# avik-pal/RegNeuralDE.jl

Hardware: AMD Instinct MI355X
Metric: training-step samples/sec + mean NFE, MNIST Neural ODE bs=512 (higher is better)
Workload: dtype f32; 1 GPU; MNIST NODE regularized (error_est), Tsit5 reltol=abstol=1.4e-8, batch 512 per GPU, 1xMI355X per rank; step = loss fwd + reverse pass through the solver + InvDecay/Momentum update; the weights train during the timed steps (mean_nfe drifts with --steps: value_fixed_weights of --full is the stationary companion); global_batch=512, parallelism=single

## Files before the change

### include/rnde.h

```cpp
#ifndef RNDE_H
#define RNDE_H
#include <stddef.h>
#include <stdint.h>

#ifdef __cplusplus
extern "C" {
#endif

#define RNDE_MAX_LAYERS 8

typedef enum {
    RNDE_OK = 0,
    RNDE_ERR_BAD_ARG = 1,
    RNDE_ERR_MAX_ATTEMPTS = 2,
    RNDE_ERR_DT_UNDERFLOW = 3,
    RNDE_ERR_NONFINITE = 4,
    RNDE_ERR_HIP = 5,
    RNDE_ERR_NO_TAPE = 6,
    RNDE_ERR_NO_DEVICE = 7
} rnde_status;

typedef enum { RNDE_ACT_IDENTITY = 0, RNDE_ACT_TANH = 1, RNDE_ACT_RELU = 2, RNDE_ACT_SIGMOID = 3, RNDE_ACT_SOFTPLUS = 4, RNDE_ACT_ELU = 5 } rnde_act;
typedef enum { RNDE_PRE_NONE = 0, RNDE_PRE_TANH = 1, RNDE_PRE_CUBE = 2 } rnde_pre_act;
typedef enum { RNDE_SOLVER_TSIT5 = 0, RNDE_SOLVER_DP5 = 1, RNDE_SOLVER_DOP853 = 2 } rnde_solver;
// ... 21 lines not shown
    int32_t wgrad_side_pct;
    int32_t stage_generic;
} rnde_node_config;

typedef struct rnde_node rnde_node;
typedef struct rnde_comm rnde_comm;

const char* rnde_version(void);
int64_t     rnde_debug_poison_allocs(void);
int64_t     rnde_debug_poison_bytes(void);
int64_t     rnde_debug_live_allocs(void);
int64_t     rnde_debug_live_bytes(void);
const char* rnde_last_error(const rnde_node* h);
int32_t     rnde_param_count(const rnde_node_config* cfg);

rnde_status rnde_node_create(const rnde_node_config* cfg, rnde_node** out);
void        rnde_node_destroy(rnde_node* h);

rnde_status rnde_node_create_tiled(const rnde_node_config* cfg, rnde_node** out);
int64_t     rnde_node_tiled_lds_bytes(const rnde_node_config* cfg);

rnde_status rnde_node_set_tracking(rnde_node* h, int32_t track_ctrl, int32_t track_initdt);
rnde_status rnde_node_tracking(const rnde_node* h, int32_t* ctrl_out, int32_t* initdt_out);

rnde_status rnde_node_tiled_reserve_saveat(rnde_node* h, int32_t max_saveat);
int32_t     rnde_node_tiled_saveat_capacity(const rnde_node* h);

rnde_status rnde_node_forward(rnde_node* h, const float* x_dev, const float* p_dev, int32_t B,
                              float t0, float t1, float* u_out_dev, int64_t* nfe_out,
                              float* saveval_host, int32_t* n_saveval_out, int32_t keep_tape,
                              void* stream);

rnde_status rnde_node_forward_saveat(rnde_node* h, const float* x_dev, const float* p_dev, int32_t B,
                                     float t0, float t1, const float* saveat_host, int32_t n_saveat,
                                     float* u_saved_dev, int64_t* nfe_out, float* saveval_host,
                                     int32_t* n_saveval_out, int32_t keep_tape, void* stream);

rnde_status rnde_node_forward_everystep(rnde_node* h, const float* x_dev, const float* p_dev, int32_t B, float t0, float t1,
                                        int32_t save_start, float* sol_out_dev, int32_t capacity, float* t_host_out, int32_t* n_out,
                                        int64_t* nfe_out, float* saveval_host, int32_t* n_saveval_out, int32_t keep_tape, void* stream);

rnde_status rnde_node_forward_replay(rnde_node* h, const float* x_dev, const float* p_dev, int32_t B,
                                     float t0, float t1, const float* steps_host, int32_t n_steps,
                                     float* u_out_dev, int64_t* nfe_out, float* saveval_host,
                                     int32_t* n_saveval_out, int32_t keep_tape, void* stream);

rnde_status rnde_debug_arm_replay(rnde_node* h, const float* steps_host, int32_t n_steps);

rnde_status rnde_node_backward(rnde_node* h, const float* u_bar_dev, const float* saveval_bar_host,
                               float* x_bar_dev, float* p_bar_dev, float* tspan_bar_host,
                               void* stream);

rnde_status rnde_node_backward_async(rnde_node* h, const float* u_bar_dev, const float* saveval_bar_host,
                                     float* x_bar_dev, float* p_bar_dev, float* tspan_bar_dev, void* stream);

rnde_status rnde_node_release_tape(rnde_node* h);

rnde_status rnde_node_forward_host(rnde_node* h, const float* x, const float* p, int32_t B, float t0,
                                   float t1, float* u_out, int64_t* nfe_out, float* saveval,
                                   int32_t* n_saveval_out, int32_t keep_tape);
rnde_status rnde_node_backward_host(rnde_node* h, const float* u_bar, const float* saveval_bar,
                                    float* x_bar, float* p_bar, float* tspan_bar);

rnde_status rnde_node_steps(rnde_node* h, float* steps_host, int32_t capacity, int32_t* n_attempts_out);
rnde_status rnde_node_attempts_ext(rnde_node* h, float* out_host, int32_t capacity, int32_t* n_attempts_out);

rnde_status rnde_debug_feval(rnde_node* h, const float* u_dev, const float* p_dev, int32_t B, float t,
                             float* out_dev, void* stream);
rnde_status rnde_debug_attempt(rnde_node* h, const float* uprev_dev, const float* k1_dev,
                               const float* p_dev, int32_t B, float t, float dt, float* k_out_dev,
                               float* unew_out_dev, float* eest_out, void* stream);
rnde_status rnde_bench_attempt(rnde_node* h, const float* x_dev, const float* p_dev, int32_t B,
                               int32_t iters, float* mean_us_out, void* stream);
rnde_status rnde_bench_attempt_taped(rnde_node* h, const float* x_dev, const float* p_dev, int32_t B,
                                     int32_t iters, float* mean_us_out, void* stream);
rnde_status rnde_bench_attempt_cold_tape(rnde_node* h, const float* x_dev, const float* p_dev, int32_t B, int32_t iters,
                                         int32_t records, float* mean_us_out, void* stream);
rnde_status rnde_node_set_timing(rnde_node* h, int32_t on);
rnde_status rnde_node_timing(rnde_node* h, float* fwd_attempts_ms, float* rev_sweep_ms, float* rev_rest_ms);
int32_t     rnde_node_last_attempts(const rnde_node* h);
int32_t     rnde_node_fallback_count(const rnde_node* h);
int32_t     rnde_node_launches_per_attempt(const rnde_node* h);
int32_t     rnde_node_one_launch_solves(const rnde_node* h);
#define RNDE_MATRIX_F32 0
#define RNDE_MATRIX_BF16X3 1
rnde_status rnde_node_set_matrix_mode(rnde_node* h, int32_t mode);
int32_t     rnde_node_matrix_mode(const rnde_node* h);

typedef struct rnde_tapes rnde_tapes;
rnde_status rnde_tapes_create(const rnde_node_config* cfg, int32_t max_tapes, rnde_tapes** out);
void        rnde_tapes_destroy(rnde_tapes* t);
const char* rnde_tapes_last_error(const rnde_tapes* t);
int32_t     rnde_tapes_in_use(const rnde_tapes* t);
rnde_node*  rnde_tapes_node(rnde_tapes* t, int32_t tape_id);
rnde_status rnde_tapes_forward(rnde_tapes* t, const float* x_dev, const float* p_dev, int32_t B, float t0, float t1, float* u_out_dev,
                               int64_t* nfe_out, float* saveval_host, int32_t* n_saveval_out, int32_t keep_tape, void* stream,
                               int32_t* tape_id_out);
rnde_status rnde_tapes_backward(rnde_tapes* t, int32_t tape_id, const float* u_bar_dev, const float* saveval_bar_host, float* x_bar_dev,
                                float* p_bar_dev, float* tspan_bar_host, void* stream);
rnde_status rnde_tapes_release(rnde_tapes* t, int32_t tape_id);

rnde_status rnde_classifier_head(rnde_node* h, const float* u_dev, const float* p3_dev, const float* y_dev,
                                 int32_t B, int32_t n_classes, float* logits_out_dev, float* u_bar_dev,
                                 float* p3_bar_dev, float* ce_out_dev, void* stream);

rnde_status rnde_node_classifier_grad(rnde_node* h, const float* x_dev, const float* p2_dev, const float* p3_dev,
                                      const float* y_dev, int32_t B, int32_t n_classes, float t0, float t1, float lambda,
                                      float* p2_bar_dev, float* p3_bar_dev, float* x_bar_dev, float* ce_out_dev,
                                      float* reg_out_host, int64_t* nfe_out, rnde_comm* comm, void* stream);

rnde_status rnde_momentum_step(float* p_dev, const float* g_dev, float* v_dev, int64_t len, int64_t n, float gamma,
                               float eta, float rho, void* stream);

rnde_status rnde_momentum_step_scaled(float* p_dev, const float* g_dev, float* v_dev, int64_t len, int64_t n, float gamma,
                                      float eta, float rho, float gscale, void* stream);
rnde_status rnde_adam_step(float* p_dev, const float* g_dev, float* m_dev, float* v_dev, int64_t len, int64_t t, float eta, float beta1,
                           float beta2, float eps, float gscale, void* stream);
rnde_status rnde_adabelief_step(float* p_dev, const float* g_dev, float* m_dev, float* s_dev, int64_t len, float eta, float beta1, float beta2,
                                float eps, float gscale, void* stream);

#define RNDE_COMM_ID_BYTES 128
rnde_status rnde_comm_unique_id(uint8_t id_out[RNDE_COMM_ID_BYTES]);
rnde_status rnde_comm_create(const uint8_t id[RNDE_COMM_ID_BYTES], int32_t rank, int32_t world, int32_t device, rnde_comm** out);
void        rnde_comm_destroy(rnde_comm* c);
int32_t     rnde_comm_world(const rnde_comm* c);
const char* rnde_comm_last_error(const rnde_comm* c);
const char* rnde_comm_library(void);
rnde_status rnde_comm_allreduce(rnde_comm* c, float* buf_dev, int64_t n, int32_t mean, void* stream);
rnde_status rnde_comm_create_local_group(int32_t world, int32_t device, rnde_comm** out);
rnde_status rnde_comm_health(rnde_comm* c);
#define RNDE_COMM_WINDOW_BYTES 64
typedef struct rnde_comm_window rnde_comm_window;
rnde_status rnde_comm_window_create(int32_t device, rnde_comm_window** win_out, uint8_t handle_out[RNDE_COMM_WINDOW_BYTES]);
void        rnde_comm_window_destroy(rnde_comm_window* w);
rnde_status rnde_comm_create_peers(rnde_comm_window* win, const uint8_t* handles, int32_t rank, int32_t world, rnde_comm** out);
const char* rnde_comm_path(const rnde_comm* c);

rnde_status rnde_node_set_coupling(rnde_node* h, rnde_comm* c, int32_t global_batch);

typedef enum { RNDE_SDE_SOSRI = 0, RNDE_SDE_SRIW1 = 1, RNDE_SDE_SOSRI2 = 2 } rnde_sde_solver;

typedef struct {
    int32_t drift_layers;
    int32_t drift_dims[RNDE_MAX_LAYERS + 1];
    int32_t drift_act[RNDE_MAX_LAYERS];
    int32_t diff_layers;
    int32_t diff_dims[RNDE_MAX_LAYERS + 1];
    int32_t diff_act[RNDE_MAX_LAYERS];
    int32_t max_batch;
    int32_t solver;
    float   reltol, abstol;
    int32_t regularize;
    int32_t cb_save_start;
    int32_t max_attempts;
    int32_t device;
    float   beta1, beta2, gamma, qmin, qmax, qoldinit, delta;
    int32_t generic;
    float   stability_size;
} rnde_nsde_config;

typedef struct rnde_nsde rnde_nsde;

int32_t     rnde_nsde_param_count(const rnde_nsde_config* cfg, int32_t* len_drift_out);
rnde_status rnde_nsde_create(const rnde_nsde_config* cfg, rnde_nsde** out);
void        rnde_nsde_destroy(rnde_nsde* h);
const char* rnde_nsde_last_error(const rnde_nsde* h);
// ... 129 lines not shown
```

### regneuralde.jl_amd/_lib.py

```python
import ctypes as C
import os

from . import build as _build

MAX_LAYERS = 8
OK, BAD_ARG, MAX_ATTEMPTS, DT_UNDERFLOW, NONFINITE, HIP_ERR, NO_TAPE, NO_DEVICE = range(8)
REG = {"none": 0, False: 0, None: 0, "error_est": 1, True: 1, "stiff_est": 2, "error_stiff_est": 3}


class NodeConfig(C.Structure):
    _fields_ = [("n_layers", C.c_int32), ("dims", C.c_int32 * (MAX_LAYERS + 1)), ("act", C.c_int32 * MAX_LAYERS),
                ("time_dep", C.c_int32), ("pre_act", C.c_int32), ("max_batch", C.c_int32), ("solver", C.c_int32),
                ("reltol", C.c_float), ("abstol", C.c_float), ("regularize", C.c_int32),
                ("cb_save_start", C.c_int32), ("track_ctrl", C.c_int32), ("track_initdt", C.c_int32),
                ("max_attempts", C.c_int32), ("device", C.c_int32), ("col_tile", C.c_int32),
                ("persist", C.c_int32), ("wgrad_side_pct", C.c_int32), ("stage_generic", C.c_int32)]


class NsdeConfig(C.Structure):
    _fields_ = [("drift_layers", C.c_int32), ("drift_dims", C.c_int32 * (MAX_LAYERS + 1)), ("drift_act", C.c_int32 * MAX_LAYERS),
                ("diff_layers", C.c_int32), ("diff_dims", C.c_int32 * (MAX_LAYERS + 1)), ("diff_act", C.c_int32 * MAX_LAYERS),
                ("max_batch", C.c_int32), ("solver", C.c_int32), ("reltol", C.c_float), ("abstol", C.c_float),
                ("regularize", C.c_int32), ("cb_save_start", C.c_int32), ("max_attempts", C.c_int32), ("device", C.c_int32),
                ("beta1", C.c_float), ("beta2", C.c_float), ("gamma", C.c_float), ("qmin", C.c_float), ("qmax", C.c_float),
# ... 126 lines not shown
    L.rnde_comm_path.argtypes = [vp]
    L.rnde_comm_path.restype = C.c_char_p
    L.rnde_tapes_create.argtypes = [C.POINTER(NodeConfig), i32, C.POINTER(vp)]
    L.rnde_tapes_destroy.argtypes = [vp]
    L.rnde_tapes_destroy.restype = None
    L.rnde_tapes_last_error.argtypes = [vp]
    L.rnde_tapes_last_error.restype = C.c_char_p
    L.rnde_tapes_in_use.argtypes = [vp]
    L.rnde_tapes_node.argtypes = [vp, i32]
    L.rnde_tapes_node.restype = vp
    L.rnde_tapes_forward.argtypes = [vp, vp, vp, i32, C.c_float, C.c_float, vp, C.POINTER(C.c_int64), fp, C.POINTER(i32), i32, vp, C.POINTER(i32)]
    L.rnde_tapes_backward.argtypes = [vp, i32, vp, fp, vp, vp, fp, vp]
    L.rnde_tapes_release.argtypes = [vp, i32]
    L.rnde_nsde_param_count.restype = i32
    L.rnde_nsde_param_count.argtypes = [C.POINTER(NsdeConfig), i32p]
    L.rnde_nsde_create.argtypes = [C.POINTER(NsdeConfig), C.POINTER(vp)]
    L.rnde_nsde_destroy.argtypes = [vp]
    L.rnde_nsde_destroy.restype = None
    L.rnde_nsde_last_error.restype = C.c_char_p
    L.rnde_nsde_last_error.argtypes = [vp]
    L.rnde_nsde_forward.argtypes = [vp, vp, vp, i32, f, f, vp, i32, u64, vp, i64p, i64p, fp, i32p, i32, vp]
    L.rnde_nsde_forward_saveat.argtypes = [vp, vp, vp, i32, f, f, vp, i32, u64, fp, i32, vp, i64p, i64p, fp, i32p, i32, vp]
    L.rnde_nsde_forward_everystep.argtypes = [vp, vp, vp, i32, f, f, vp, i32, u64, i32, vp, i32, fp, i32p, i64p, i64p, fp, i32p, i32, vp]
    L.rnde_nsde_forward_replay.argtypes = [vp, vp, vp, i32, f, f, vp, i32, fp, i32, vp, i64p, i64p, fp, i32p, i32, vp]
    L.rnde_nsde_backward.argtypes = [vp, vp, fp, vp, vp, vp]
    L.rnde_nsde_backward_async.argtypes = [vp, vp, fp, vp, vp, vp]
    L.rnde_nsde_classifier_head.argtypes = [vp, vp, vp, vp, i32, i32, vp, vp, vp, vp, vp]
    L.rnde_nsde_classifier_grad.argtypes = [vp, vp, vp, vp, vp, i32, i32, f, f, vp, i32, C.c_uint64, f, vp, vp, vp, vp, fp, C.POINTER(C.c_int64), C.POINTER(C.c_int64), vp]
    L.rnde_nsde_steps.argtypes = [vp, fp, i32, i32p, i32p]
    L.rnde_nsde_debug_attempt.argtypes = [vp, vp, vp, i32, f, vp, vp, vp, vp, fp, vp]
    L.rnde_nsde_set_pre_act.argtypes = [vp, i32, i32]
    L.rnde_nsde_moment_grad.argtypes = [vp, vp, vp, i32, f, f, vp, i32, u64, fp, i32, vp, vp, f, vp, vp, vp, fp, i64p, i64p, vp]
    L.rnde_nsde_timing.argtypes = [vp, fp, fp, i32p, i32p]
    L.rnde_normal_fill.argtypes = [vp, C.c_int64, u64, u64, vp]
    L.rnde_latent_create.argtypes = [C.POINTER(LatentConfig), C.POINTER(vp)]
    L.rnde_latent_destroy.argtypes = [vp]
    L.rnde_latent_destroy.restype = None
    L.rnde_latent_last_error.argtypes = [vp]
    L.rnde_latent_last_error.restype = C.c_char_p
    L.rnde_latent_param_counts.argtypes = [i32p, i32p, i32p]
    L.rnde_latent_param_counts.restype = None
    L.rnde_latent_encode.argtypes = [vp, vp, vp, vp, vp, i32, i32, vp, vp, vp, vp]
    L.rnde_latent_decode_loss.argtypes = [vp, vp, vp, vp, i32, i32, vp, vp, vp, vp]
    L.rnde_latent_encode_backward.argtypes = [vp, vp, f, vp, vp, vp, vp, vp, vp]
    L.rnde_adamax_step.argtypes = [vp, vp, vp, vp, C.c_int64, C.c_int64, f, f, f, f, f, f, vp]
    L.rnde_ffjord_param_count.restype = i32
    L.rnde_ffjord_param_count.argtypes = [C.POINTER(FfjordConfig)]
    L.rnde_ffjord_create.argtypes = [C.POINTER(FfjordConfig), C.POINTER(vp)]
    L.rnde_ffjord_destroy.argtypes = [vp]
    L.rnde_ffjord_destroy.restype = None
    L.rnde_ffjord_last_error.argtypes = [vp]
    L.rnde_ffjord_last_error.restype = C.c_char_p
    L.rnde_ffjord_forward.argtypes = [vp, vp, vp, vp, i32, f, f, u64, vp, vp, i64p, fp, i32p, i32, vp]
    L.rnde_ffjord_forward_replay.argtypes = [vp, vp, vp, vp, i32, f, f, u64, fp, i32, vp, vp, i64p, fp, i32p, i32, vp]
    L.rnde_ffjord_steps.argtypes = [vp, fp, i32, i32p]
    L.rnde_ffjord_backward.argtypes = [vp, vp, fp, vp, vp, vp]
    L.rnde_ffjord_sample.argtypes = [vp, vp, vp, i32, f, f, u64, vp, vp]
    L.rnde_ffjord_debug_feval.argtypes = [vp, vp, vp, vp, i32, f, i32, vp, vp]
    L.rnde_ffjord_timing.argtypes = [vp, fp, fp, i32p, i32p]
    L.rnde_ffjord_create_tiled.argtypes = [C.POINTER(FfjordConfig), C.POINTER(vp)]
    L.rnde_ffjord_engine.restype = i32
    L.rnde_ffjord_engine.argtypes = [vp]
    L.rnde_ffjord_forward_kinetic.argtypes = [vp, vp, vp, vp, i32, f, f, u64, vp, vp, vp, i64p, i32, vp]
    L.rnde_ffjord_forward_kinetic_replay.argtypes = [vp, vp, vp, vp, i32, f, f, u64, fp, i32, vp, vp, vp, i64p, i32, vp]
    L.rnde_ffjord_backward_kinetic.argtypes = [vp, vp, vp, vp, vp, vp]
    L.rnde_ffjord_debug_feval_kinetic.argtypes = [vp, vp, vp, vp, i32, f, vp, vp]
    L.rnde_ffjord_step_log.argtypes = [vp, fp, i32, i32p]
    L.rnde_ffjord_chain_param_count.restype = i32
    L.rnde_ffjord_chain_param_count.argtypes = [C.POINTER(FfjordChainConfig)]
    L.rnde_ffjord_create_chain.argtypes = [C.POINTER(FfjordChainConfig), C.POINTER(vp)]
    L.rnde_ffjord_forward_exact.argtypes = [vp, vp, vp, i32, f, f, vp, vp, i64p, fp, i32p, i32, vp]
    L.rnde_ffjord_forward_exact_replay.argtypes = [vp, vp, vp, i32, f, f, fp, i32, vp, vp, i64p, fp, i32p, i32, vp]
    L.rnde_ffjord_set_track_ctrl.argtypes = [vp, i32]
    L.rnde_ffjord_track_ctrl.restype = i32
    L.rnde_ffjord_track_ctrl.argtypes = [vp]
    _lib = L
    return L


EXPORTS = ["rnde_version", "rnde_debug_poison_allocs", "rnde_debug_poison_bytes", "rnde_debug_live_allocs", "rnde_debug_live_bytes", "rnde_last_error", "rnde_param_count", "rnde_node_create", "rnde_node_destroy",
           "rnde_node_forward", "rnde_node_forward_saveat", "rnde_node_forward_everystep", "rnde_node_forward_replay", "rnde_node_backward", "rnde_node_backward_async", "rnde_node_release_tape", "rnde_node_forward_host",
           "rnde_node_backward_host", "rnde_node_steps", "rnde_debug_feval", "rnde_debug_attempt",
           "rnde_bench_attempt", "rnde_bench_attempt_taped", "rnde_bench_attempt_cold_tape", "rnde_node_set_timing", "rnde_node_timing", "rnde_node_last_attempts", "rnde_node_fallback_count",
           "rnde_node_launches_per_attempt", "rnde_node_one_launch_solves", "rnde_node_set_matrix_mode", "rnde_node_matrix_mode", "rnde_classifier_head", "rnde_node_classifier_grad", "rnde_momentum_step", "rnde_momentum_step_scaled", "rnde_adam_step",
           "rnde_comm_unique_id", "rnde_comm_create", "rnde_comm_destroy", "rnde_comm_world", "rnde_comm_last_error", "rnde_comm_library", "rnde_comm_allreduce", "rnde_comm_create_local_group", "rnde_comm_health", "rnde_comm_window_create", "rnde_comm_window_destroy", "rnde_comm_create_peers", "rnde_comm_path", "rnde_node_set_coupling", "rnde_tapes_create", "rnde_tapes_destroy", "rnde_tapes_last_error", "rnde_tapes_in_use", "rnde_tapes_node", "rnde_tapes_forward", "rnde_tapes_backward", "rnde_tapes_release",
           "rnde_nsde_param_count", "rnde_nsde_create", "rnde_nsde_destroy", "rnde_nsde_last_error", "rnde_nsde_forward",
           "rnde_nsde_forward_saveat", "rnde_nsde_forward_everystep", "rnde_nsde_forward_replay", "rnde_nsde_backward", "rnde_nsde_backward_async", "rnde_nsde_classifier_head", "rnde_nsde_classifier_grad", "rnde_nsde_steps", "rnde_nsde_debug_attempt", "rnde_nsde_set_pre_act", "rnde_nsde_moment_grad", "rnde_moment_loss", "rnde_adabelief_step", "rnde_nsde_timing", "rnde_normal_fill", "rnde_latent_create", "rnde_latent_destroy", "rnde_latent_last_error", "rnde_latent_param_counts", "rnde_latent_encode",
           "rnde_latent_decode_loss", "rnde_latent_encode_backward", "rnde_adamax_step",
           "rnde_ffjord_param_count", "rnde_ffjord_create", "rnde_ffjord_destroy", "rnde_ffjord_last_error", "rnde_ffjord_forward",
           "rnde_ffjord_forward_replay", "rnde_ffjord_steps", "rnde_ffjord_backward", "rnde_ffjord_sample", "rnde_ffjord_debug_feval",
           "rnde_ffjord_timing", "rnde_ffjord_create_tiled", "rnde_ffjord_engine", "rnde_ffjord_forward_kinetic",
           "rnde_ffjord_forward_kinetic_replay", "rnde_ffjord_backward_kinetic", "rnde_ffjord_debug_feval_kinetic", "rnde_ffjord_step_log",
           "rnde_ffjord_chain_param_count", "rnde_ffjord_create_chain", "rnde_ffjord_forward_exact", "rnde_ffjord_forward_exact_replay",
           "rnde_ffjord_set_track_ctrl", "rnde_ffjord_track_ctrl",
           "rnde_node_create_tiled", "rnde_node_tiled_lds_bytes", "rnde_node_set_tracking", "rnde_node_tracking", "rnde_node_attempts_ext",
           "rnde_node_tiled_reserve_saveat", "rnde_node_tiled_saveat_capacity", "rnde_debug_arm_replay"]


def check(h, status):
    if status != OK:
        msg = lib().rnde_last_error(h).decode() if h else lib().rnde_last_error(None).decode()
        raise RndeError(status, msg)


def check_latent(h, status):
    if status != OK:
        raise RndeError(status, lib().rnde_latent_last_error(h if h else None).decode())


def check_ffjord(h, status):
    if status != OK:
        raise RndeError(status, lib().rnde_ffjord_last_error(h if h else None).decode())


def check_nsde(h, status):
    if status != OK:
        raise RndeError(status, lib().rnde_nsde_last_error(h if h else None).decode())
```

### regneuralde.jl_amd/csrc/rnde.hip

```cpp
#include "rnde_node.h"

static thread_local std::string g_create_err;
void rnde_set_create_error(const std::string& msg) { g_create_err = msg; }
extern "C" const char* rnde_version(void) { return "rnde 0.1.0 (gfx950)"; }
extern "C" int64_t rnde_debug_poison_allocs(void) { return (int64_t)rnde_g_poison_allocs.load(); }
extern "C" int64_t rnde_debug_poison_bytes(void) { return (int64_t)rnde_g_poison_bytes.load(); }
extern "C" int64_t rnde_debug_live_allocs(void) { return (int64_t)rnde_g_live_allocs.load(); }
extern "C" int64_t rnde_debug_live_bytes(void) { return (int64_t)rnde_g_live_bytes.load(); }
extern "C" const char* rnde_last_error(const rnde_node* h) { return h ? h->err.c_str() : g_create_err.c_str(); }

extern "C" int32_t rnde_param_count(const rnde_node_config* c) {
    int n = 0;
    for (int l = 0; l < c->n_layers; ++l) n += (c->dims[l] + (c->time_dep ? 1 : 0)) * c->dims[l + 1] + c->dims[l + 1];
    return n;
}

StepParams make_params(rnde_node* h, const float* x, int B, float t0, float t1, int tape) {
    StepParams P{};
    P.x = x;
    P.f0 = h->f0; P.h0 = h->h0; P.u1 = h->u1; P.f1 = h->f1; P.h1 = h->h1;
    P.arena = h->arena; P.rec_stride = h->rec_stride;
    P.ctl = h->ctl; P.ctl_final = h->ctl_final; P.meta = h->meta; P.initrec = h->initrec;
    P.errpart = h->errpart; P.initpart = h->initpart; P.dbg_out = nullptr;
    P.D = h->D; P.H = h->H; P.B = B; P.Bn = h->couple ? h->couple_batch : B;
// ... 356 lines not shown
        } else h->x3 = 0;
    }
    h->predicted = 12;
    *out = hold.release();
    return RNDE_OK;
}

extern "C" void rnde_node_destroy(rnde_node* h) {
    if (!h) return;
    node_tiled_destroy(h);
    delete h;
}

rnde_status couple_sum(rnde_node* h, float* partials, long long count, hipStream_t s) {
    if (!h->couple) return RNDE_OK;
    const rnde_status st = rnde_comm_allreduce(h->couple, partials, count, 0, (void*)s);
    if (st != RNDE_OK) h->err = std::string("coupled controller: ") + rnde_comm_last_error(h->couple);
    return st;
}
extern "C" rnde_status rnde_node_set_coupling(rnde_node* h, rnde_comm* c, int32_t global_batch) {
    if (!h) return RNDE_ERR_BAD_ARG;
    RNDE_TILED_REFUSE(h, "rnde_node_set_coupling is not served (one controller over several shards: the stage engine and the chain engine's multi-wave kernels, rnde_node_create)");
    if (!c) { h->couple = nullptr; h->couple_batch = 0; h->couple_world = 1; return RNDE_OK; }
    const int world = rnde_comm_world(c);
    if (h->engine != 2 && !(h->engine == 3 && h->mw)) { h->err = "coupled controller: the stage engine (MNIST form, col_tile 0 or 16) and the chain engine's multi-wave kernels only"; return RNDE_ERR_BAD_ARG; }
    if (global_batch < world || world < 1) { h->err = "coupled controller: global_batch must cover every rank"; return RNDE_ERR_BAD_ARG; }
    h->couple = c; h->couple_batch = global_batch; h->couple_world = world;
    return RNDE_OK;
}

static rnde_status ensure_arena(rnde_node* h, long long recs) {
    HIPCHK(h, h->arena.reserve((size_t)recs * h->rec_stride));
    return RNDE_OK;
}

static StageParams make_stage_params(rnde_node* h, const StepParams& P, const float* p_dev) {
    StageParams Q{};
    Q.F = P; Q.p = p_dev; Q.pwB = h->spwB; Q.pwD = h->spwD; Q.slab = h->slab2;
    Q.MT = h->sMT; Q.WT = h->sWT; Q.R = h->sR; Q.C = P.Bpad / 16; Q.HT = h->sHT; Q.K2b = h->sK2b; Q.Bpad16 = P.Bpad;
    return Q;
}
template <int ACT2, int MODE>
static hipError_t launch_stage_t(rnde_node* h, const StageParams& Q, int n, int s, hipStream_t st) {
    hipLaunchKernelGGL((rnde_stage_kernel<ACT2, MODE>), dim3(Q.R * Q.C), dim3(64 * Q.WT), h->stage_lds, st, Q, n, s);
    return hipGetLastError();
}
template <int MODE>
static hipError_t launch_stage(rnde_node* h, const StageParams& Q, int n, int s, hipStream_t st) {
    return h->act2 ? launch_stage_t<1, MODE>(h, Q, n, s, st) : launch_stage_t<0, MODE>(h, Q, n, s, st);
}
hipError_t stage_pack(rnde_node* h, const float* p, f32x4* dst, int which, int MTrows, int Kb, hipStream_t st) {
    const long long total = (long long)MTrows * Kb * 64;
    const int grid = (int)std::min<long long>((total + 255) / 256, 1024);
    hipLaunchKernelGGL(rnde_stage_pack_kernel, dim3(grid), dim3(256), 0, st, p, dst, which, h->D, h->H, MTrows, Kb);
    return hipGetLastError();
}
static rnde_status x3_pack(rnde_node* h, const float* p_dev, bool with_rev, hipStream_t s) {
    h->x3_fwd = false;
    if (!(h->x3 && h->x3B && h->x3D && h->persist == 1 && !h->stage_generic)) return RNDE_OK;
    HIPCHK(h, rnde_launch_x3_pack(p_dev, h->x3B, h->x3D, with_rev ? h->x3Bt : nullptr, with_rev ? h->x3Dt : nullptr, h->D, h->H, h->sMT, h->sWT, h->sR, h->sHT, s));
    h->x3_fwd = true;
    h->x3_packed = with_rev;
    return RNDE_OK;
}
static rnde_status stage_pack_weights(rnde_node* h, const float* p_dev, hipStream_t s) {
    HIPCHK(h, stage_pack(h, p_dev, h->spwB, 0, h->sMT, h->sK2b, s));
    HIPCHK(h, stage_pack(h, p_dev, h->spwD, 1, h->sHT, h->sMT, s));
    return x3_pack(h, p_dev, false, s);
}
rnde_status stage_pack_all(rnde_node* h, const float* p_dev, hipStream_t s, const float* x_src, long long x_floats) {
    PackJobs J{};
    int n = 0;
    auto add = [&](void* dst, long long total, int kind, int which, int kdim, const float* src = nullptr) { J.j[n++] = PackJob{dst, src, total, kind, which, kdim, 0}; };
    add(h->spwB, (long long)h->sMT * h->sK2b * 64, 0, 0, h->sK2b);
    add(h->spwD, (long long)h->sHT * h->sMT * 64, 0, 1, h->sMT);
    add(h->spwBt, (long long)h->sMT * h->sKHb * 64, 0, 2, h->sKHb);
    add(h->spwDt, (long long)h->sHT * h->sMT * 64, 0, 3, h->sMT);
    auto add_copy = [&](float* dst, const float* src, long long floats) {
        const bool v4 = floats % 4 == 0 && ((uintptr_t)dst % 16 == 0) && ((uintptr_t)(src ? src : p_dev) % 16 == 0);
        add(dst, v4 ? floats / 4 : floats, v4 ? 3 : 2, 0, 0, src);
    };
    add_copy(h->pcopy, nullptr, (long long)h->P);
    if (x_src) add_copy(h->xcopy, x_src, x_floats);
    long long most = 0;
    for (int i = 0; i < n; ++i) most = std::max(most, J.j[i].total);
    const int grid = (int)std::min<long long>((most + 255) / 256, 256);
    hipLaunchKernelGGL(rnde_pack_all_kernel, dim3(grid, n), dim3(256), 0, s, p_dev, J, h->D, h->H);
    HIPCHK(h, hipGetLastError());
    h->rev_packed = true;
    return x3_pack(h, p_dev, true, s);
}
hipError_t slab_prepare(rnde_node* h, int Bpad, hipStream_t s) {
    if (h->tslab_Bpad == Bpad) return hipSuccess;
    h->tslab_Bpad = Bpad;
    return hipMemsetAsync(h->tslab, 0xFF, h->tslab_bytes, s);
}
static bool stage_two_tile(const rnde_node* h, const StageParams& Q) {
    const bool fix = Q.WT == 7 && Q.HT == 7 && Q.K2b == 7 && Q.MT == 49 && Q.R == 7 && h->D == 784 && h->H == 100 && !h->stage_generic;
    return h->persist == 1 && fix && Q.C % 2 == 0 && h->persist2 != 0 && (Q.C >= kPersist2MinTiles || h->persist2 >= 1);
}
static bool stage_epart_reduce(const rnde_node* h, const StageParams& Q) {
    return stage_two_tile(h, Q) && Q.F.nwg >= 896 && !getenv("RNDE_NO_EPART_REDUCE");
}
static hipError_t stage_attempt(rnde_node* h, const StageParams& Q, int n, hipStream_t s) {
    if (h->persist == 1) {
        PersistSync Y{h->tslab, h->pabort, h->pxcc, h->persist_spins};
        if (hipError_t e = slab_prepare(h, Q.Bpad16, s); e != hipSuccess) return e;
        const dim3 grid(8 * Q.R * ((Q.C + 7) / 8));
        const bool fix = Q.WT == 7 && Q.HT == 7 && Q.K2b == 7 && Q.MT == 49 && Q.R == 7 && h->D == 784 && h->H == 100 && !h->stage_generic;
        static const bool x3_over_mt = !(getenv("RNDE_X3_MT") && atoi(getenv("RNDE_X3_MT")) == 0);
        if (stage_two_tile(h, Q)) {
            const dim3 grid2(8 * Q.R * ((Q.C / 2 + 7) / 8));
            if (h->x3_fwd && x3_over_mt) {
                const size_t xlds2 = sizeof(float) * ((size_t)2 * 2 * kX3ImageFloats + 32 * 3);
                if (h->act2) hipLaunchKernelGGL((rnde_stage_attempt_mt_kernel<1, 2, 1>), grid2, dim3(64 * 7), xlds2, s, Q, n, Y, (const void*)h->x3B, (const void*)h->x3D);
                else hipLaunchKernelGGL((rnde_stage_attempt_mt_kernel<0, 2, 1>), grid2, dim3(64 * 7), xlds2, s, Q, n, Y, (const void*)h->x3B, (const void*)h->x3D);
                return hipGetLastError();
            }
            const size_t lds2 = sizeof(float) * (2 * 2 * 16 * (16 * 7 + 4) + 32 * 3);
            if (h->act2) hipLaunchKernelGGL((rnde_stage_attempt_mt_kernel<1, 2>), grid2, dim3(64 * 7), lds2, s, Q, n, Y, (const void*)nullptr, (const void*)nullptr);
            else hipLaunchKernelGGL((rnde_stage_attempt_mt_kernel<0, 2>), grid2, dim3(64 * 7), lds2, s, Q, n, Y, (const void*)nullptr, (const void*)nullptr);
            return hipGetLastError();
        }
        if (fix && h->x3_fwd) {
            const size_t xlds = sizeof(float) * ((size_t)2 * kX3ImageFloats + 64);
            if (h->act2) hipLaunchKernelGGL((rnde_stage_attempt_kernel<1, 1, 1>), grid, dim3(64 * 7), xlds, s, Q, n, Y, (const void*)h->x3B, (const void*)h->x3D);
            else hipLaunchKernelGGL((rnde_stage_attempt_kernel<0, 1, 1>), grid, dim3(64 * 7), xlds, s, Q, n, Y, (const void*)h->x3B, (const void*)h->x3D);
        } else if (fix) {
            if (h->act2) hipLaunchKernelGGL((rnde_stage_attempt_kernel<1, 1>), grid, dim3(64 * Q.WT), h->stage_lds, s, Q, n, Y, (const void*)nullptr, (const void*)nullptr);
            else hipLaunchKernelGGL((rnde_stage_attempt_kernel<0, 1>), grid, dim3(64 * Q.WT), h->stage_lds, s, Q, n, Y, (const void*)nullptr, (const void*)nullptr);
        } else if (h->act2) hipLaunchKernelGGL((rnde_stage_attempt_kernel<1, 0>), grid, dim3(64 * Q.WT), h->stage_lds, s, Q, n, Y, (const void*)nullptr, (const void*)nullptr);
        else hipLaunchKernelGGL((rnde_stage_attempt_kernel<0, 0>), grid, dim3(64 * Q.WT), h->stage_lds, s, Q, n, Y, (const void*)nullptr, (const void*)nullptr);
        return hipGetLastError();
    }
    hipError_t e = launch_stage<SM_START>(h, Q, n, 0, s);
    for (int st = 1; st <= 5 && e == hipSuccess; ++st) e = launch_stage<SM_STAGE>(h, Q, n, st, s);
    if (e == hipSuccess) e = launch_stage<SM_LAST>(h, Q, n, 6, s);
    return e;
}

bool bsweep_failed(rnde_node* h, hipStream_t s) {
    if (!h->pending_bsweep) return false;
    h->pending_bsweep = false;
    const MeetVerdict v = meet_verdict(h->h_mw_bchk, h->bsweep_nt, h->bsweep_global);
    if (v == MEET_OK) return false;
    fprintf(stderr, "[rnde] chain engine: one-launch reverse sweep abandoned (%s); one launch per reversed attempt for the next %d solves\n",
            v == MEET_TIMED_OUT ? "a meeting timed out" : "workgroups pinned by block index landed on different XCDs", h->mw_retry_after);
    h->mw_bsweep = -1; h->mw_clean = 0; ++h->persist_fallbacks;
    h->mw_meet.clear_abort(s);
    h->h_mw_bchk[0] = 0;
    return true;
}

static rnde_status forward_core(rnde_node* h, const float* x_dev, const float* p_dev, int32_t B, float t0, float t1,
                                float* u_out_dev, const float* saveat_host, int32_t n_saveat, float* sv_out_dev,
                                int64_t* nfe_out, float* saveval_host, int32_t* n_saveval_out, int32_t keep_tape, void* stream);

void persist_check_enqueue(rnde_node* h, int grid, hipStream_t s) {
    if (h->persist != 1) return;
    h->h_pchk[0] = 1;
    if (hipMemcpyAsync(h->h_pchk, h->pabort, 8, hipMemcpyDeviceToHost, s) != hipSuccess) return;
    (void)hipMemcpyAsync(h->h_pchk + 2, h->pxcc, (size_t)grid * 4, hipMemcpyDeviceToHost, s);
}
bool persist_check_result(rnde_node* h, int C, int R, hipStream_t s) {
    if (h->persist != 1) return false;
    bool bad = h->h_pchk[0] != 0;
    for (int ct = 0; ct < C && !bad; ++ct)
        for (int rb = 1; rb < R; ++rb) if (h->h_pchk[2 + rb * C + ct] != h->h_pchk[2 + ct]) { bad = true; break; }
    if (bad) {
        fprintf(stderr, "[rnde] persistent attempt kernel suspended (%s); using the multi-launch kernels for the next %d solves\n",
                h->h_pchk[0] ? "hand-off timed out" : "column tile spans XCDs", h->persist_retry_after);
        h->persist = -1; h->persist_clean = 0; ++h->persist_fallbacks;
// ... 367 lines not shown
    return RNDE_OK;
}

extern "C" rnde_status rnde_node_forward_everystep(rnde_node* h, const float* x_dev, const float* p_dev, int32_t B, float t0, float t1, int32_t save_start,
                                                   float* sol_out_dev, int32_t capacity, float* t_host_out, int32_t* n_out, int64_t* nfe_out,
                                                   float* saveval_host, int32_t* n_saveval_out, int32_t keep_tape, void* stream) {
    if (!h || !n_out || !sol_out_dev || capacity < 1) return RNDE_ERR_BAD_ARG;
    if (rnde_node_tiled_saveat_capacity(h) == 0)
        RNDE_TILED_REFUSE(h, "rnde_node_forward_everystep is not served (the end state only; save_everystep runs on the engines of rnde_node_create)");
    rnde_status st = forward_impl(h, x_dev, p_dev, B, t0, t1, nullptr, nullptr, 0, nullptr, nullptr, nullptr, nullptr, 0, stream);
    if (st != RNDE_OK) return st;
    std::vector<float> times;
    if (save_start) times.push_back(t0);
    for (int i = 0; i < h->n_att; ++i) {
        const StepMeta& m = h->h_meta[i];
        if (m.flags & F_ACCEPT) { float tn = m.t + m.dt; if (tn > t1) tn = t1; times.push_back(tn); }
    }
    *n_out = (int32_t)times.size();
    if ((int)times.size() > capacity) { h->err = "rnde_node_forward_everystep: more accepted steps than the output has room for"; return RNDE_ERR_BAD_ARG; }
    if (t_host_out) memcpy(t_host_out, times.data(), times.size() * sizeof(float));
    st = forward_impl(h, x_dev, p_dev, B, t0, t1, nullptr, times.data(), (int32_t)times.size(), sol_out_dev, nfe_out, saveval_host, n_saveval_out, keep_tape, stream);
    if (st != RNDE_OK) return st;
    size_t k = save_start ? 1 : 0;
    for (int i = 0; i < h->n_att; ++i) {
        const StepMeta& m = h->h_meta[i];
        if (!(m.flags & F_ACCEPT)) continue;
        float tn = m.t + m.dt; if (tn > t1) tn = t1;
        if (k >= times.size() || times[k] != tn) { h->err = "rnde_node_forward_everystep: the saving solve did not retrace the steps of the first one"; return RNDE_ERR_HIP; }
        ++k;
    }
    if (k != times.size()) { h->err = "rnde_node_forward_everystep: the saving solve took fewer accepted steps than the first one"; return RNDE_ERR_HIP; }
    return RNDE_OK;
}

extern "C" rnde_status rnde_node_steps(rnde_node* h, float* steps_host, int32_t capacity, int32_t* n_out) {
    if (!h) return RNDE_ERR_BAD_ARG;
    const int n = std::min(capacity, h->n_att);
    for (int i = 0; i < n; ++i) {
        steps_host[4 * i + 0] = h->h_meta[i].t; steps_host[4 * i + 1] = h->h_meta[i].dt;
        steps_host[4 * i + 2] = h->h_meta[i].eest; steps_host[4 * i + 3] = (h->h_meta[i].flags & F_ACCEPT) ? 1.f : 0.f;
    }
    if (n_out) *n_out = h->n_att;
    return RNDE_OK;
}

extern "C" rnde_status rnde_node_attempts_ext(rnde_node* h, float* out_host, int32_t capacity, int32_t* n_out) {
    if (!h || !n_out) return RNDE_ERR_BAD_ARG;
    *n_out = h->n_att;
    if (out_host) {
        if (capacity < h->n_att) { h->err = "rnde_node_attempts_ext: capacity below the attempt count"; return RNDE_ERR_BAD_ARG; }
        for (int i = 0; i < h->n_att; ++i) {
            const StepMeta& m = h->h_meta[i];
            float* o = out_host + 6 * (size_t)i;
            o[0] = m.t; o[1] = m.dt; o[2] = m.dtp_in; o[3] = m.eest; o[4] = (m.flags & F_ACCEPT) ? 1.f : 0.f; o[5] = m.q;
        }
    }
    return RNDE_OK;
}

extern "C" rnde_status rnde_node_set_timing(rnde_node* h, int32_t on) {
    if (!h) return RNDE_ERR_BAD_ARG;
    if (on) for (auto& e : h->tev) HIPCHK(h, e.create());
    h->timing = on ? 1 : 0; h->tev_fwd = h->tev_bwd = false;
    return RNDE_OK;
}
extern "C" rnde_status rnde_node_timing(rnde_node* h, float* fwd_attempts_ms, float* rev_sweep_ms, float* rev_rest_ms) {
    if (h && h->engine == 4) return node_tiled_timing(h, fwd_attempts_ms, rev_sweep_ms, rev_rest_ms);
    if (!h || !h->timing) return RNDE_ERR_BAD_ARG;
    float a = -1.f, b = -1.f, c = -1.f;
    if (h->tev_fwd) { HIPCHK(h, hipEventSynchronize(h->tev[1])); HIPCHK(h, hipEventElapsedTime(&a, h->tev[0], h->tev[1])); }
    if (h->tev_bwd) {
        HIPCHK(h, hipEventSynchronize(h->tev[4]));
        HIPCHK(h, hipEventElapsedTime(&b, h->tev[2], h->tev[3])); HIPCHK(h, hipEventElapsedTime(&c, h->tev[3], h->tev[4]));
    }
    if (fwd_attempts_ms) *fwd_attempts_ms = a;
    if (rev_sweep_ms) *rev_sweep_ms = b;
    if (rev_rest_ms) *rev_rest_ms = c;
    return RNDE_OK;
}
extern "C" int32_t rnde_node_last_attempts(const rnde_node* h) { return h ? h->n_att : 0; }
extern "C" int32_t rnde_node_fallback_count(const rnde_node* h) { return h ? h->persist_fallbacks : 0; }

extern "C" int32_t rnde_node_one_launch_solves(const rnde_node* h) { return h ? h->one_launch_solves : 0; }
extern "C" rnde_status rnde_node_set_matrix_mode(rnde_node* h, int32_t mode) {
    if (!h) return RNDE_ERR_BAD_ARG;
    if (mode != RNDE_MATRIX_F32 && mode != RNDE_MATRIX_BF16X3) { h->err = "matrix mode: 0 (fp32-input MFMA) or 1 (bf16x3 on the matrix cores)"; return RNDE_ERR_BAD_ARG; }
    if (mode == RNDE_MATRIX_BF16X3) RNDE_TILED_REFUSE(h, "rnde_node_set_matrix_mode(h, 1) is not served (its layer products are the fp32-input MFMA, mode 0; bf16x3 serves the MNIST form on the stage engine)");
    h->x3 = (mode == RNDE_MATRIX_BF16X3 && h->x3B && h->x3D) ? 1 : 0;
    return RNDE_OK;
}
extern "C" int32_t rnde_node_matrix_mode(const rnde_node* h) { return (h && h->x3 && h->x3B && h->x3D) ? RNDE_MATRIX_BF16X3 : RNDE_MATRIX_F32; }
extern "C" int32_t rnde_node_launches_per_attempt(const rnde_node* h) {
    if (!h) return 0;
    return (h->engine == 2 && h->persist != 1) ? 7 : 1;
}

extern "C" rnde_status rnde_node_release_tape(rnde_node* h) {
    if (!h) return RNDE_ERR_BAD_ARG;
    h->have_tape = false;
    return RNDE_OK;
}

extern "C" rnde_status rnde_node_forward_host(rnde_node* h, const float* x, const float* p, int32_t B, float t0, float t1,
                                              float* u_out, int64_t* nfe_out, float* saveval, int32_t* n_saveval_out,
                                              int32_t keep_tape) {
    if (!h) return RNDE_ERR_BAD_ARG;
    DevBuf<float> xd, pd, ud;
    const size_t nb = (size_t)h->D * B * 4;
    HIPCHK(h, xd.alloc(nb / 4)); HIPCHK(h, ud.alloc(nb / 4)); HIPCHK(h, pd.alloc((size_t)h->P));
    HIPCHK(h, hipMemcpy(xd, x, nb, hipMemcpyHostToDevice)); HIPCHK(h, hipMemcpy(pd, p, (size_t)h->P * 4, hipMemcpyHostToDevice));
    rnde_status st = rnde_node_forward(h, xd, pd, B, t0, t1, ud, nfe_out, saveval, n_saveval_out, keep_tape, nullptr);
    if (st == RNDE_OK || st == RNDE_ERR_MAX_ATTEMPTS) hipMemcpy(u_out, ud, nb, hipMemcpyDeviceToHost);
    return st;
}

extern "C" rnde_status rnde_debug_feval(rnde_node* h, const float* u_dev, const float* p_dev, int32_t B, float t,
                                        float* out_dev, void* stream) {
    if (!h || B < 1 || B > h->cfg.max_batch) return RNDE_ERR_BAD_ARG;
    if (h->engine == 4) return node_tiled_feval(h, u_dev, p_dev, B, t, out_dev, stream);
    hipStream_t s = (hipStream_t)stream;
    StepParams P = make_params(h, u_dev, B, 0.f, 1.f, 0);
    P.forced = 1; P.forced_t = t; P.dbg_out = out_dev;
    if (h->engine == 3) {
        rnde_status st3 = chain_pack(h, p_dev, s);
        if (st3 != RNDE_OK) return st3;
        if (h->mw) HIPCHK(h, launch_mw<MW_FEVAL>(h, make_mw_params(h, P), 0, s));
        else HIPCHK(h, launch_chain<CM_FEVAL>(h, make_chain_params(h, P), 0, nullptr, s));
        HIPCHK(h, hipStreamSynchronize(s));
        return RNDE_OK;
    }
    if (h->engine == 2) {
        rnde_status st2 = stage_pack_weights(h, p_dev, s);
        if (st2 != RNDE_OK) return st2;
        StageParams SQ = make_stage_params(h, P, p_dev);
        HIPCHK(h, launch_stage<SM_FEVAL1>(h, SQ, 0, 0, s));
        HIPCHK(h, launch_stage<SM_FEVAL2>(h, SQ, 0, 0, s));
        HIPCHK(h, hipStreamSynchronize(s));
        return RNDE_OK;
    }
    h->err = "rnde_debug_feval: unknown engine";
    return RNDE_ERR_BAD_ARG;
}

extern "C" rnde_status rnde_debug_attempt(rnde_node* h, const float* uprev_dev, const float* k1_dev, const float* p_dev,
                                          int32_t B, float t, float dt, float* k_out_dev, float* unew_out_dev,
                                          float* eest_out, void* stream) {
    if (!h || B < 1 || B > h->cfg.max_batch) return RNDE_ERR_BAD_ARG;
    RNDE_TILED_REFUSE(h, "rnde_debug_attempt is not served (its solve is one launch with no single-attempt entry; rnde_node_forward_replay runs a given attempt sequence)");
    hipStream_t s = (hipStream_t)stream;
    h->have_tape = false;
    StepParams P = make_params(h, uprev_dev, B, 0.f, 1.f, 0);
    P.forced = 1; P.forced_t = t; P.forced_dt = dt;
    if (h->engine == 3) {
        rnde_status st3 = chain_pack(h, p_dev, s);
        if (st3 != RNDE_OK) return st3;
        const ChainParams CQ = make_chain_params(h, P);
        const int nks = h->NKD;
        HIPCHK(h, chain_convert(k1_dev, h->f0, h->D, B, CQ.ntiles, nks, 0, s));
        if (h->mw) { HIPCHK(h, launch_mw<MW_STEP>(h, make_mw_params(h, P), 0, s)); HIPCHK(h, launch_mw<MW_FINISH>(h, make_mw_params(h, P), 1, s)); }
        else { HIPCHK(h, launch_chain<CM_STEP>(h, CQ, 0, nullptr, s)); HIPCHK(h, launch_chain<CM_FINISH>(h, CQ, 1, nullptr, s)); }
        HIPCHK(h, hipMemcpyAsync(h->h_ctl, h->ctl_final, sizeof(StepState), hipMemcpyDeviceToHost, s));
        const ChainRec CL{(long long)CQ.ntiles * nks * 64, h->rk_S};
        for (int sidx = 2; sidx <= h->rk_S; ++sidx)
            HIPCHK(h, chain_convert(h->arena + CL.k(sidx), k_out_dev + (size_t)(sidx - 2) * h->D * B, h->D, B, CQ.ntiles, nks, 1, s));
        HIPCHK(h, chain_convert(h->arena + CL.unew(), unew_out_dev, h->D, B, CQ.ntiles, nks, 1, s));
        HIPCHK(h, hipStreamSynchronize(s));
// ... 129 lines not shown
```

### regneuralde.jl_amd/csrc/rnde_binit_stage.h

```cpp
#pragma once
#include "rnde_bstage.h"

namespace rnde {

template <int ACT2, int STEP>
__global__ __launch_bounds__(64 * kSMaxW) void rnde_binit_stage_kernel(const BStageParams Q) {
#pragma clang fp contract(off)
    const BwdParams& Bq = Q.B;
    const StepParams& P = Bq.F;
    extern __shared__ __attribute__((aligned(16))) float smem[];
    const int KZ = 16 * Q.KHb + 4, KG = 16 * Q.WT + 4;
    float* ZL = smem;
    float* GL = ZL + kSCB * KZ;
    float* RED = GL + kSCB * KG;
    const int tid = threadIdx.x, lane = tid & 63;
    const int w = __builtin_amdgcn_readfirstlane(tid >> 6);
    const int rb = blockIdx.x / Q.C, ct = blockIdx.x - rb * Q.C;
    const int wg = blockIdx.x;
    const int col = lane & 15, gcol = ct * kSCB + col;
    const bool colok = gcol < P.B;
    const bool vec = (P.D & 3) == 0;
    const bool writer = (blockIdx.x == 0 && tid == 0);
    const int T = rb * Q.WT + w;
    const int r0 = 16 * T + 4 * (lane >> 4);
    const bool tile_ok = T < Q.MT;
    const long long A = (long long)P.D * P.Bpad, HB = (long long)P.H * P.Bpad;
    const size_t co = (size_t)gcol * P.D;
    const double N = (double)P.D * (double)P.Bn;
    const InitRec ir = *P.initrec;
    const float dt0 = ir.dt0;
    constexpr bool kD = (STEP == 0 || STEP == 2);
    constexpr int kPhase = STEP < 2 ? 1 : 2;
    constexpr int par = STEP < 2 ? 0 : 1;

    float dot = 0.f, tau = 0.f;
    if constexpr (kD) {
        f32x4 wD[kSMaxW];
#pragma unroll
        for (int kb = 0; kb < kSMaxW; ++kb)
            if (kb < Q.WT && w < Q.HT && rb * Q.WT + kb < Q.MT) wD[kb] = Q.pwDt[((size_t)w * Q.MT + rb * Q.WT + kb) * 64 + lane];
        f32x4 xv = {0.f, 0.f, 0.f, 0.f}, f0v = xv, f1v = xv, ub1 = xv, Uv = xv, K1v = xv;
        if (tile_ok) {
            xv = ld4(P.x + co, r0, P.D, colok, P.xvec != 0);
            f0v = ld4(P.f0 + co, r0, P.D, true, vec);
            f1v = ld4(P.f1 + co, r0, P.D, true, vec);
            if constexpr (kPhase == 2) {
                ub1 = ld4(Bq.UB1 + co, r0, P.D, true, vec);
                Uv = ld4(Bq.U + co, r0, P.D, true, vec);
                K1v = ld4(Bq.K1 + co, r0, P.D, true, vec);
            }
        }
        f32x4 v = {0.f, 0.f, 0.f, 0.f};
        if constexpr (kPhase == 1) {
            double tb, dtpb, qoldb, t1b, t0b;
            finish_attempt_scalars(Bq, 0, lane, tb, dtpb, qoldb, t1b, t0b);
            const double dtb = Bq.track_initdt ? dtpb : 0.0;
            double dt0b = 0, d1b = 0, d2b = 0;
            if (ir.sel == 2) { t1b += dtb; t0b -= dtb; }
            else if (ir.sel == 0) dt0b += 100.0 * dtb;
            else if (!ir.dt1_const) {
                const double mm = ir.max_is_d2 ? (double)ir.d2 : (double)ir.d1;
                const double mb = dtb * (-0.2) * (double)ir.dt1 / mm;
                if (ir.max_is_d2) d2b += mb; else d1b += mb;
            } else if (dt0 * 1e-3f > 1e-6f) dt0b += 1e-3 * dtb;
            const double n2 = (double)ir.d2 * (double)dt0, n2b = d2b / (double)dt0;
            dt0b += -d2b * (double)ir.d2 / (double)dt0;
            const double coef_w = n2 > 0 ? n2b / (N * n2) : 0.0;
            if (writer) { IBState b; b.tb = tb; b.t1b = t1b; b.t0b = t0b; b.dt0b = dt0b; b.d1b = d1b; b.d2b = d2b; b.coef_w = coef_w; b.pad = 0; Bq.ibstate[0] = b; }
            const float cw = (float)coef_w;
            if (tile_ok) {
#pragma unroll
                for (int i = 0; i < 4; ++i) {
                    const float sk = P.abstol + fabsf(xv[i]) * P.reltol;
                    const float wv = (f1v[i] - f0v[i]) / sk;
                    const float f1b = (colok && r0 + i < P.D ? cw * wv : 0.f) / sk;
                    v[i] = ACT2 ? f1b * (1.f - f1v[i] * f1v[i]) : f1b;
                }
                st4(Bq.zi2 + A + co, r0, P.D, true, vec, v);
            }
        } else {
            const IBState ib = Bq.ibstate[0];
            double dot1 = 0, tau1 = 0;
            for (int i = lane; i < P.nwg; i += 64) { dot1 += (double)Bq.ipart[4 * i]; tau1 += (double)Bq.ipart[4 * i + 1]; }
            dot1 = wave_sum_d(dot1); tau1 = wave_sum_d(tau1);
            double dt0b = ib.dt0b + tau1 + dot1, t0b = ib.t0b + tau1, t1b = ib.t1b, d1b = ib.d1b, d0b = 0;
            if (ir.dt0_clamped) { t1b += dt0b; t0b -= dt0b; }
            else if (!ir.dt0_const) { d0b = dt0b / (100.0 * (double)ir.d1); d1b += -dt0b * (double)dt0 / (double)ir.d1; }
            const float cv = ir.d1 > 0.f ? (float)(d1b / (N * (double)ir.d1)) : 0.f;
            const float cz = ir.d0 > 0.f ? (float)(d0b / (N * (double)ir.d0)) : 0.f;
            const float cw = (float)ib.coef_w;
            if (writer) { IBState b = ib; b.t1b = t1b; b.t0b = t0b; Bq.ibstate[1] = b; }
            if (tile_ok) {
                f32x4 u0b = {0.f, 0.f, 0.f, 0.f};
#pragma unroll
                for (int i = 0; i < 4; ++i) {
                    const bool ok = colok && r0 + i < P.D;
                    const float sk = P.abstol + fabsf(xv[i]) * P.reltol;
                    const float wv = (f1v[i] - f0v[i]) / sk, vv = f0v[i] / sk, z = xv[i] / sk;
                    const float wb = ok ? cw * wv : 0.f, vb = ok ? cv * vv : 0.f, zb = ok ? cz * z : 0.f;
                    const float skb = -(wb * wv + vb * vv + zb * z) / sk;
                    const float f0b = K1v[i] + dt0 * ub1[i] + (vb - wb) / sk;
                    u0b[i] = Uv[i] + ub1[i] + zb / sk + skb * P.reltol * sgnf(xv[i]);
                    if (Bq.sv_ubar0 && ok) u0b[i] += Bq.sv_ubar0[((size_t)gcol * Bq.sv_T) * P.D + r0 + i];
                    v[i] = ACT2 ? f0b * (1.f - f0v[i] * f0v[i]) : f0b;
                }
                st4(Bq.zi2 + co, r0, P.D, true, vec, v);
                st_tile(Bq.xbar + co, r0, P.D, colok, false, u0b);
            }
        }
#pragma unroll
        for (int i = 0; i < 4; ++i) GL[col * KG + kperm(16 * w + 4 * (lane >> 4) + i)] = tile_ok ? v[i] : 0.f;
        __syncthreads();
        f32x4* sl = (f32x4*)Q.slab + ((((size_t)par * Q.C + ct) * Q.R + rb) * Q.HT) * 64;
        const float* gbp = GL + col * KG + 4 * (lane >> 4);
        f32x4 bg[kSMaxW];
#pragma unroll
        for (int kb = 0; kb < kSMaxW; ++kb) if (kb < Q.WT) bg[kb] = *(const f32x4*)(gbp + 16 * kb);
        if (w < Q.HT) {
            f32x4 acc0 = {0.f, 0.f, 0.f, 0.f}, acc1 = {0.f, 0.f, 0.f, 0.f};
#pragma unroll
            for (int kb = 0; kb < kSMaxW; ++kb) {
                if (kb < Q.WT && rb * Q.WT + kb < Q.MT) {
                    acc0 = mfma16(wD[kb][0], bg[kb][0], acc0);
                    acc1 = mfma16(wD[kb][1], bg[kb][1], acc1);
                    acc0 = mfma16(wD[kb][2], bg[kb][2], acc0);
                    acc1 = mfma16(wD[kb][3], bg[kb][3], acc1);
                }
            }
            sl[(size_t)w * 64 + lane] = acc0 + acc1;
        }
        for (int ht = w + Q.WT; ht < Q.HT; ht += Q.WT) {
            f32x4 acc0 = {0.f, 0.f, 0.f, 0.f}, acc1 = {0.f, 0.f, 0.f, 0.f};
#pragma unroll
            for (int kb = 0; kb < kSMaxW; ++kb) {
                if (kb < Q.WT && rb * Q.WT + kb < Q.MT) {
                    const f32x4 a = Q.pwDt[((size_t)ht * Q.MT + rb * Q.WT + kb) * 64 + lane];
                    acc0 = mfma16(a[0], bg[kb][0], acc0);
                    acc1 = mfma16(a[1], bg[kb][1], acc1);
                    acc0 = mfma16(a[2], bg[kb][2], acc0);
                    acc1 = mfma16(a[3], bg[kb][3], acc1);
                }
            }
            sl[(size_t)ht * 64 + lane] = acc0 + acc1;
        }
        return;
    } else {
        f32x4 wB[kSMaxHT];
#pragma unroll
        for (int kb = 0; kb < kSMaxHT; ++kb)
            if (kb < Q.KHb && tile_ok) wB[kb] = Q.pwBt[((size_t)T * Q.KHb + kb) * 64 + lane];
        const float* hsrc = kPhase == 1 ? P.h1 : P.h0;
        float* z1dst = kPhase == 1 ? Bq.zi1 + HB : Bq.zi1;
        const float* W1t = Q.p + (size_t)P.H * P.D;
        const f32x4* sl = (const f32x4*)Q.slab + (((size_t)par * Q.C + ct) * Q.R) * Q.HT * 64;
        f32x4 f0v = {0.f, 0.f, 0.f, 0.f};
        if (kPhase == 1 && tile_ok) f0v = ld4(P.f0 + co, r0, P.D, true, vec);
        for (int ht = w; ht < Q.HT; ht += Q.WT) {
            f32x4 z = {0.f, 0.f, 0.f, 0.f};
            for (int r = 0; r < Q.R; ++r) z += sl[((size_t)r * Q.HT + ht) * 64 + lane];
            const int h0 = 16 * ht + 4 * (lane >> 4);
#pragma unroll
            for (int i = 0; i < 4; ++i) {
                const int hr = h0 + i;
                float zv = 0.f;
                if (hr < P.H) {
                    const float hv = hsrc[(size_t)gcol * P.H + hr];
                    zv = z[i] * (1.f - hv * hv);
                    if (rb == 0) { z1dst[(size_t)gcol * P.H + hr] = zv; tau += W1t[hr] * zv; }
                } else if (hr == P.H) {
                    if (rb == 0) tau += z[i];
                }
                if (hr < 16 * Q.KHb) ZL[col * KZ + kperm(hr)] = zv;
            }
        }
        if (Q.KHb > Q.HT) {
            for (int i = tid; i < kSCB * 16 * Q.KHb; i += blockDim.x) {
                const int c = i / (16 * Q.KHb), k = i - c * 16 * Q.KHb;
                if (k >= 16 * Q.HT) ZL[c * KZ + kperm(k)] = 0.f;
            }
        }
        __syncthreads();
        f32x4 gb = {0.f, 0.f, 0.f, 0.f};
        if (tile_ok) {
            f32x4 acc0 = {0.f, 0.f, 0.f, 0.f}, acc1 = {0.f, 0.f, 0.f, 0.f};
            const float* zb = ZL + col * KZ + 4 * (lane >> 4);
            f32x4 bf[kSMaxHT];
#pragma unroll
            for (int kb = 0; kb < kSMaxHT; ++kb) if (kb < Q.KHb) bf[kb] = *(const f32x4*)(zb + 16 * kb);
#pragma unroll
            for (int kb = 0; kb < kSMaxHT; ++kb) {
                if (kb < Q.KHb) {
                    acc0 = mfma16(wB[kb][0], bf[kb][0], acc0);
                    acc1 = mfma16(wB[kb][1], bf[kb][1], acc1);
                    acc0 = mfma16(wB[kb][2], bf[kb][2], acc0);
                    acc1 = mfma16(wB[kb][3], bf[kb][3], acc1);
                }
            }
            gb = acc0 + acc1;
#pragma unroll
            for (int i = 0; i < 4; ++i) if (r0 + i >= P.D) gb[i] = 0.f;
            if constexpr (kPhase == 1) {
                st4(Bq.UB1 + co, r0, P.D, true, vec, gb);
#pragma unroll
                for (int i = 0; i < 4; ++i) dot += gb[i] * f0v[i];
            } else {
                const f32x4 u0b = ld_tile(Bq.xbar + co, r0, P.D, colok, false);
                st_tile(Bq.xbar + co, r0, P.D, colok, false, u0b + gb);
            }
        }
        if (!colok) tau = 0.f;
        dot = wave_sum_f(dot); tau = wave_sum_f(tau);
        __syncthreads();
        if (lane == 0) { RED[w] = dot; RED[8 + w] = tau; }
        __syncthreads();
        if (tid == 0) {
            float sa = 0.f, ta = 0.f;
            for (int i = 0; i < Q.WT; ++i) { sa += RED[i]; ta += RED[8 + i]; }
            if constexpr (kPhase == 1) { float* o = Bq.ipart + (size_t)wg * 4; o[0] = sa; o[1] = ta; o[2] = 0.f; o[3] = 0.f; }
            else { float* o = Bq.ipart + ((size_t)P.nwg + wg) * 4; o[0] = ta; o[1] = 0.f; o[2] = 0.f; o[3] = 0.f; }
        }
    }
}

}
```

### regneuralde.jl_amd/csrc/rnde_bwd.h

```cpp
#pragma once
#include "rnde_fwd.h"

namespace rnde {

struct BState {
    double tb_pre, dtb_pre, qoldb, t1b, t0b, pad[3];
};
struct IBState {
    double tb, t1b, t0b, dt0b, d1b, d2b, coef_w, pad;
};
struct EvalDesc {
    const float* Z;
    const float* X;
    float t;
    int pad;
};

struct BwdParams {
    StepParams F;
    float* U; float* K1; float* UB1;
    float* zi2; float* zi1;
    const float* svb_att;
    BState* bstate;
    IBState* ibstate;
// ... 353 lines not shown
        for (int s = 0; s < KC / 4; ++s) {
            __builtin_amdgcn_sched_barrier(0);
            if (s + 1 < KC / 4) operands(s + 1, a[(s + 1) & 1], bq[(s + 1) & 1]);
            if ((s == 1 || s == 5) && s == (w < 4 ? 1 : 5) && step + 1 < total_steps) stage_dma((step + 1) & 1);
#pragma unroll
            for (int i = 0; i < 3; ++i)
#pragma unroll
                for (int n = 0; n < 7; ++n) acc[i][n] = mfma16(a[s & 1][i], bq[s & 1][n], acc[i][n]);
            if (has3) {
#pragma unroll
                for (int n = 0; n < 7; ++n) acc[3][n] = mfma16(a[s & 1][3], bq[s & 1][n], acc[3][n]);
            }
        }
        wait_vm<0>();
        __syncthreads();
    }
    float* out = slab + (size_t)chunk * M * (Nx + 2);
#pragma unroll
    for (int i = 0; i < 4; ++i) {
        if (w + 7 * i < ntile) {
#pragma unroll
            for (int n = 0; n < 7; ++n) {
                const int sr = 16 * n + mrow;
#pragma unroll
                for (int q = 0; q < 4; ++q) {
                    const int tr = row_lo + 16 * (w + 7 * i) + 4 * kk + q;
                    if (tr < TR && sr < SR) out[TALL_IS_Z ? (size_t)sr * M + tr : (size_t)tr * M + sr] = acc[i][n][q];
                }
            }
        }
    }
}

static __global__ void rnde_wgrad_reduce(const float* __restrict__ slab, int n_chunks, int per_group, long long len, float* __restrict__ out) {
    const int c0 = blockIdx.y * per_group, c1 = min(n_chunks, c0 + per_group);
    float* o = out + (size_t)blockIdx.y * len;
    for (long long i = blockIdx.x * (long long)blockDim.x + threadIdx.x; i < len; i += (long long)gridDim.x * blockDim.x) {
        float s = 0.f;
        int c = c0;
        for (; c + 8 <= c1; c += 8) {
            float v[8];
#pragma unroll
            for (int j = 0; j < 8; ++j) v[j] = __builtin_nontemporal_load(slab + (size_t)(c + j) * len + i);
#pragma unroll
            for (int j = 0; j < 8; ++j) s += v[j];
        }
        for (; c < c1; ++c) s += __builtin_nontemporal_load(slab + (size_t)c * len + i);
        o[i] = s;
    }
}
static inline hipError_t launch_wgrad_reduce(const float* slab, int chunks, long long len, float* slab_r, float* out, hipStream_t s) {
    const int grid = (int)((len + 255) / 256 < 2048 ? (len + 255) / 256 : 2048);
    if (chunks <= 16) {
        hipLaunchKernelGGL(rnde_wgrad_reduce, dim3(grid, 1), dim3(256), 0, s, slab, chunks, chunks, len, out);
    } else {
        const int per_group = (chunks + 15) / 16, groups = (chunks + per_group - 1) / per_group;
        hipLaunchKernelGGL(rnde_wgrad_reduce, dim3(grid, groups), dim3(256), 0, s, slab, chunks, per_group, len, slab_r);
        hipLaunchKernelGGL(rnde_wgrad_reduce, dim3(grid, 1), dim3(256), 0, s, (const float*)slab_r, groups, groups, len, out);
    }
    return hipGetLastError();
}

struct ReduceJob { const float* slab; float* out; long long len; int n_chunks, per_group; };
struct ReducePair { ReduceJob j[2]; };
static __global__ void rnde_wgrad_reduce_pair(const ReducePair R) {
    const ReduceJob J = R.j[blockIdx.z];
    const int c0 = blockIdx.y * J.per_group, c1 = min(J.n_chunks, c0 + J.per_group);
    if (c0 >= c1) return;
    float* o = J.out + (size_t)blockIdx.y * J.len;
    for (long long i = blockIdx.x * (long long)blockDim.x + threadIdx.x; i < J.len; i += (long long)gridDim.x * blockDim.x) {
        float s = 0.f;
        int c = c0;
        for (; c + 8 <= c1; c += 8) {
            float v[8];
#pragma unroll
            for (int j = 0; j < 8; ++j) v[j] = __builtin_nontemporal_load(J.slab + (size_t)(c + j) * J.len + i);
#pragma unroll
            for (int j = 0; j < 8; ++j) s += v[j];
        }
        for (; c < c1; ++c) s += __builtin_nontemporal_load(J.slab + (size_t)c * J.len + i);
        o[i] = s;
    }
}

}
```

### regneuralde.jl_amd/csrc/rnde_node.h

```cpp
#pragma once
#include "../../include/rnde.h"
#include "rnde_alloc.h"
#include "rnde_fwd.h"
#include "rnde_bwd.h"
#include "rnde_stage.h"
#include "rnde_bstage.h"
#include "rnde_stage_persist2.h"
#include "rnde_bstage_persist.h"
#include "rnde_solve_sync.h"
#include "rnde_meet.h"
#include "rnde_binit_stage.h"
#include "rnde_head.h"
#include "rnde_chain.h"
#include "rk_tables.h"
#include "rnde_bchain.h"
#include "rnde_chainmw.h"
#include "rnde_bchainmw.h"
#include "rnde_rev_plan.h"

#include <chrono>
#include <algorithm>
#include <atomic>
#include <cmath>
#include <cstdlib>
#include <cstdio>
#include <cstring>
#include <functional>
#include <memory>
#include <string>
#include <type_traits>
#include <vector>


extern "C" hipError_t rnde_launch_stage_solve(const void* stage_params, const void* persist_sync, const void* solve_sync, int act2, int x3, hipStream_t s);
extern "C" hipError_t rnde_launch_x3_pack(const float* p, void* x3B, void* x3D, void* x3Bt, void* x3Dt, int D, int H, int MT, int WT, int R, int HT, hipStream_t s);
using namespace rnde;

struct rnde_node {
    rnde_node_config cfg{};
    int D = 0, H = 0, P = 0, BT = 8, act2 = 1;
    int Bpad_max = 0, nwg_max = 0;
    Stream wstream;
    Event wevents[66];
    Event tev[5];
    Event ev_host;
    int engine = 0;
    struct rnde_node_tiled* tiled = nullptr;
    ChainGeo cg{}; DevBuf<float> cfrags; int NKD = 0, chain_alt = 0;
    int chain_ga = 0;
    size_t chain_lds_f = 0, chain_lds_b = 0;
    rnde_comm* couple = nullptr; int couple_batch = 0, couple_world = 1;
    int rk_tab = 0; RkTab rk{};
    int mw_clean = 0, mw_retry_after = 8;
    int mw_solve = 1; MeetRes mw_meet;
    int mw_bsweep = 1; DevBuf<int> mw_bargs; PinBuf<int> h_mw_bargs; PinBuf<unsigned> h_mw_bchk; bool pending_bsweep = false; int bsweep_nt = 0; bool bsweep_global = false;
    int rk_S = 7, rk_order = 5;
    int mw_lat = 0;
    int mw = 0; MwGeo mg{}; DevBuf<float> mw_tab; DevBuf<float> mw_slab; long long mw_slab_evals = 0; size_t mw_lds_f = 0, mw_lds_b = 0;
    DevBuf<float> cslab; DevBuf<float> ev_t; PinBuf<float> h_ev_t;
    int sMT = 0, sWT = 0, sR = 0, sHT = 0, sK2b = 0, sKHb = 0;
    DevBuf<f32x4> spwB, spwD, spwBt, spwDt;
    DevBuf<float> slab2;
    size_t stage_lds = 0;
    DevBuf<float> head_ws;
    std::function<rnde_status(hipStream_t)> after_solve; bool rev_packed = false;
    DevBuf<float> cg_ws; std::vector<float> cg_sv;
    DevBuf<float> sv_t_dev; std::vector<float> saveat;
    DevBuf<float> replay_dev; const float* replay_host = nullptr; int n_replay = 0;
    std::vector<float> replay_armed;
    int wgrad_side_pct = 30, stage_generic = 0;
    int persist_clean = 0, persist_retry_after = 8, persist_fallbacks = 0;
    int persist2 = -1;
    int persist = 0, persist_spins = kPersistMaxSpins; int tslab_Bpad = -1; size_t tslab_bytes = 0; DevBuf<float> tslab; unsigned *pabort = nullptr, *pxcc = nullptr; unsigned* h_pchk = nullptr;
    int stage_solve = 1; MeetRes s_meet; int one_launch_solves = 0;
    int x3 = 0; DevBuf<unsigned char> x3B, x3D, x3Bt, x3Dt; bool x3_packed = false, x3_fwd = false;
    DevBuf<float> f0, h0, u1, f1, h1, arena;
    DevBuf<float> xcopy;
    long long rec_stride = 0;
    DevBuf<float> pcopy;
    DevBuf<StepState> ctl;
    DevBuf<unsigned char> mbox; PinBuf<unsigned char> h_mbox; size_t mbox_meta_off = 0;
    StepState* ctl_final = nullptr;
    StepMeta* meta = nullptr;
    InitRec* initrec = nullptr;
    StepState* h_ctl = nullptr;
    StepMeta* h_meta = nullptr;
    InitRec* h_init = nullptr;
    DevBuf<StepState> own_ctl_final; DevBuf<StepMeta> own_meta; DevBuf<InitRec> own_initrec;
    PinBuf<StepState> own_h_ctl; PinBuf<StepMeta> own_h_meta; PinBuf<InitRec> own_h_init;
    DevBuf<float> errpart, initpart;
    BwdBuffers bw;
    PinBuf<float> h_scal;
    int B = 0, Bpad = 0, nwg = 0, n_att = 0, predicted = 0;
    float t0 = 0, t1 = 0;
    bool have_tape = false;
    bool pending_bwd = false;
    DevBuf<float> diag_buf;
    std::vector<int> sv_index;
    int n_saveval = 0;
    int timing = 0; bool tev_fwd = false, tev_bwd = false;
    std::string err;
};

#define HIPCHK(h, call)                                                                              \
    do {                                                                                             \
        hipError_t e__ = (call);                                                                     \
        if (e__ != hipSuccess) {                                                                     \
            (h)->err = std::string(#call) + ": " + hipGetErrorString(e__);                           \
            return RNDE_ERR_HIP;                                                                     \
        }                                                                                            \
    } while (0)

void rnde_set_create_error(const std::string& msg);
void node_tiled_destroy(rnde_node* h);
rnde_status node_tiled_forward(rnde_node* h, const float* x_dev, const float* p_dev, int32_t B, float t0, float t1, float* u_out_dev,
                               const float* saveat_host, int32_t n_saveat, float* sv_out_dev, int64_t* nfe_out, float* saveval_host,
                               int32_t* n_saveval_out, int32_t keep_tape, void* stream);
rnde_status node_tiled_backward(rnde_node* h, const float* u_bar_dev, const float* saveval_bar_host, float* x_bar_dev, float* p_bar_dev,
                                float* tspan_bar_host, void* stream);
rnde_status node_tiled_feval(rnde_node* h, const float* u_dev, const float* p_dev, int32_t B, float t, float* out_dev, void* stream);
rnde_status node_tiled_timing(rnde_node* h, float* fwd_ms, float* rev_sweep_ms, float* rev_rest_ms);
#define RNDE_TILED_REFUSE(h, what)                                                                                                       \
    do {                                                                                                                                 \
        if ((h) && (h)->engine == 4) {                                                                                                   \
            (h)->err = std::string("TrackedNeuralODE tiled engine: ") + what;                                                            \
            return RNDE_ERR_BAD_ARG;                                                                                                     \
        }                                                                                                                                \
    } while (0)

template <int V> using IC = std::integral_constant<int, V>;
template <class F>
static auto chain_variant(const rnde_node* h, F&& f) {
    if (h->chain_ga) switch (h->NKD) {
        case 4: return f(IC<4>{}, IC<2>{});
        case 8: return f(IC<8>{}, IC<2>{});
        default: return f(IC<16>{}, IC<2>{});
    }
    switch (h->NKD) {
        case 4: return f(IC<4>{}, IC<0>{});
        case 8: return h->chain_alt ? f(IC<8>{}, IC<1>{}) : f(IC<8>{}, IC<0>{});
        default: return f(IC<16>{}, IC<0>{});
    }
}
template <class F>
static auto mw_variant(const rnde_node* h, F&& f) {
    auto by_nr = [&](auto tab, auto lat) {
        switch (h->NKD) {
            case 4: return f(IC<1>{}, tab, lat);
            case 8: return f(IC<2>{}, tab, lat);
            default: return f(IC<4>{}, tab, lat);
        }
    };
    auto by_tab = [&](auto lat) { return h->rk_tab == 2 ? by_nr(IC<2>{}, lat) : (h->rk_tab ? by_nr(IC<1>{}, lat) : by_nr(IC<0>{}, lat)); };
    if (h->chain_ga) return by_tab(IC<2>{});
    if (h->rk_tab != 2 && h->mw_lat) return h->rk_tab ? f(IC<2>{}, IC<1>{}, IC<1>{}) : f(IC<2>{}, IC<0>{}, IC<1>{});
    return by_tab(IC<0>{});
}

static const rnde_status RNDE_INTERNAL_RETRY = static_cast<rnde_status>(100);
StepParams make_params(rnde_node* h, const float* x, int B, float t0, float t1, int tape);
MwParams make_mw_params(rnde_node* h, const StepParams& P);
ChainParams make_chain_params(rnde_node* h, const StepParams& P);
rnde_status couple_sum(rnde_node* h, float* partials, long long count, hipStream_t s);
hipError_t stage_pack(rnde_node* h, const float* p, f32x4* dst, int which, int MTrows, int Kb, hipStream_t st);
rnde_status stage_pack_all(rnde_node* h, const float* p_dev, hipStream_t s, const float* x_src = nullptr, long long x_floats = 0);
hipError_t slab_prepare(rnde_node* h, int Bpad, hipStream_t s);
void persist_check_enqueue(rnde_node* h, int grid, hipStream_t s);
bool persist_check_result(rnde_node* h, int C, int R, hipStream_t s);
bool bsweep_failed(rnde_node* h, hipStream_t s);
rnde_status forward_impl(rnde_node* h, const float* x_dev, const float* p_dev, int32_t B, float t0, float t1,
                         float* u_out_dev, const float* saveat_host, int32_t n_saveat, float* sv_out_dev,
                         int64_t* nfe_out, float* saveval_host, int32_t* n_saveval_out, int32_t keep_tape, void* stream);
```

### regneuralde.jl_amd/csrc/rnde_reverse.hip

```cpp
#include "rnde_node.h"
#include "rnde_wgradx.h"

static rnde_status chain_bwd_run(rnde_node* h, const float* u_bar_dev, const float* saveval_bar_host, float* x_bar_dev,
                                 float* p_bar_dev, float* tspan_bar_host, hipStream_t s, bool sync = true, float* tspan_bar_dev = nullptr);
static rnde_status bwd_run(rnde_node* h, const float* u_bar_dev, const float* saveval_bar_host, float* x_bar_dev,
                           float* p_bar_dev, float* tspan_bar_host, hipStream_t s, bool sync = true, float* tspan_bar_dev = nullptr);


extern "C" rnde_status rnde_node_backward_async(rnde_node* h, const float* u_bar_dev, const float* saveval_bar_host, float* x_bar_dev,
                                                float* p_bar_dev, float* tspan_bar_dev, void* stream) {
    if (!h) return RNDE_ERR_BAD_ARG;
    RNDE_TILED_REFUSE(h, "rnde_node_backward_async is not served (rnde_node_backward runs its reverse sweep and waits for it)");
    if (!h->have_tape) { h->err = "no recorded forward"; return RNDE_ERR_NO_TAPE; }
    if (h->engine == 3) return chain_bwd_run(h, u_bar_dev, saveval_bar_host, x_bar_dev, p_bar_dev, nullptr, (hipStream_t)stream, false, tspan_bar_dev);
    return bwd_run(h, u_bar_dev, saveval_bar_host, x_bar_dev, p_bar_dev, nullptr, (hipStream_t)stream, false, tspan_bar_dev);
}

extern "C" rnde_status rnde_node_backward(rnde_node* h, const float* u_bar_dev, const float* saveval_bar_host,
                                          float* x_bar_dev, float* p_bar_dev, float* tspan_bar_host, void* stream) {
    if (!h) return RNDE_ERR_BAD_ARG;
    if (!h->have_tape) { h->err = "no recorded forward"; return RNDE_ERR_NO_TAPE; }
    if (h->engine == 4) return node_tiled_backward(h, u_bar_dev, saveval_bar_host, x_bar_dev, p_bar_dev, tspan_bar_host, stream);
    if (h->engine == 3) return chain_bwd_run(h, u_bar_dev, saveval_bar_host, x_bar_dev, p_bar_dev, tspan_bar_host, (hipStream_t)stream);
    return bwd_run(h, u_bar_dev, saveval_bar_host, x_bar_dev, p_bar_dev, tspan_bar_host, (hipStream_t)stream);
}
extern "C" rnde_status rnde_node_backward_host(rnde_node* h, const float* u_bar, const float* saveval_bar, float* x_bar,
                                               float* p_bar, float* tspan_bar) {
    if (!h) return RNDE_ERR_BAD_ARG;
    DevBuf<float> ub, xb, pb;
    const size_t nb = (size_t)h->D * h->B * 4;
    HIPCHK(h, ub.alloc(nb / 4)); HIPCHK(h, xb.alloc(nb / 4)); HIPCHK(h, pb.alloc((size_t)h->P));
    HIPCHK(h, hipMemcpy(ub, u_bar, nb, hipMemcpyHostToDevice));
    rnde_status st = rnde_node_backward(h, ub, saveval_bar, xb, pb, tspan_bar, nullptr);
    if (st == RNDE_OK) { hipMemcpy(x_bar, xb, nb, hipMemcpyDeviceToHost); hipMemcpy(p_bar, pb, (size_t)h->P * 4, hipMemcpyDeviceToHost); }
    return st;
}

static rnde_status bwd_prepare(rnde_node* h) {
    BwdBuffers& b = h->bw;
    if (b.ready) return RNDE_OK;
    const size_t A = (size_t)h->D * h->Bpad_max, HB = (size_t)h->H * h->Bpad_max;
    const int cap = h->cfg.max_attempts;
    HIPCHK(h, b.U.reserve(A)); HIPCHK(h, b.K1.reserve(A)); HIPCHK(h, b.UB1.reserve(A));
    HIPCHK(h, b.zi2.reserve(2 * A)); HIPCHK(h, b.zi1.reserve(2 * HB));
    HIPCHK(h, b.svb_att.reserve((size_t)cap));
    HIPCHK(h, b.bstate_mem.reserve(2 * sizeof(BState) + 64)); b.bstate = (BState*)b.bstate_mem.get(); HIPCHK(h, b.ibstate.reserve(2));
    HIPCHK(h, b.bpart.reserve((size_t)(2 * h->nwg_max + 256) * 4)); HIPCHK(h, b.ipart.reserve((size_t)2 * h->nwg_max * 4));
    HIPCHK(h, b.tspan_out.reserve(2));
    const size_t nev = (size_t)6 * cap + 2;
    const size_t desc_blob = 2 * nev * sizeof(EvalDesc) + (size_t)cap * 4 + 64;
    HIPCHK(h, b.ev1_mem.reserve(desc_blob)); b.ev1 = (EvalDesc*)b.ev1_mem.get(); HIPCHK(h, b.ev2.reserve(nev));
    HIPCHK(h, b.h_ev1_mem.reserve(desc_blob)); b.h_ev1 = (EvalDesc*)b.h_ev1_mem.get(); HIPCHK(h, b.h_ev2.reserve(nev));
    HIPCHK(h, b.h_svb.reserve((size_t)cap));
    const size_t seg = std::max((size_t)h->H * (h->D + 2), (size_t)h->D * (h->H + 2));
    b.slab_floats = seg * 256;
    HIPCHK(h, b.slab.reserve(2 * b.slab_floats));
    HIPCHK(h, b.slab_r.reserve(2 * 16 * seg));
    if (!h->wstream) {
        int prio_least = 0, prio_greatest = 0;
        (void)hipDeviceGetStreamPriorityRange(&prio_least, &prio_greatest);
        HIPCHK(h, hipStreamCreateWithPriority(&h->wstream.s, hipStreamNonBlocking, prio_least));
        for (auto& e : h->wevents) HIPCHK(h, e.create(hipEventDisableTiming));
    }
    HIPCHK(h, b.UTB.reserve(A)); HIPCHK(h, b.UNB.reserve(A)); HIPCHK(h, b.UPB0.reserve(A));
    HIPCHK(h, b.GB.reserve(15 * A));
    b.ready = true;
    return RNDE_OK;
}

static bool wgrad3_ok(int M, int Nx) {
    const bool tall = M >= Nx;
    const int wide = tall ? M : Nx + 2, narrow = tall ? Nx + 2 : M;
    return getenv("RNDE_WGRAD_LEGACY") == nullptr && getenv("RNDE_WGRAD_V2") == nullptr && M % 4 == 0 && Nx % 4 == 0 && wide > 656 &&
           wide <= 800 && narrow <= 112;
}
using WgradKern = decltype(&rnde_wgrad3_kernel<true>);
static rnde_status launch_wgrad_part(rnde_node* h, const EvalDesc* ev, int n_evals, int per_chunk, int M, int Nx, int Bpad,
                                     float* slab, int* chunk_cursor, hipStream_t s, int max_chunks = 0) {
    if (n_evals <= 0) return RNDE_OK;
    const int mtiles = (M + 31) / 32, ntiles = (Nx + 2 + 31) / 32;
    const bool tall = M >= Nx;
    const int MB = tall ? 2 : 4, NB = tall ? 4 : 2;
    const int blocks = ((mtiles + MB - 1) / MB) * ((ntiles + NB - 1) / NB);
    const long long len = (long long)M * (Nx + 2);
    const int chunks = (n_evals + per_chunk - 1) / per_chunk;
    float* dst = slab + (size_t)(*chunk_cursor) * len;
    static const bool legacy = getenv("RNDE_WGRAD_LEGACY") != nullptr;
    const bool fits = tall ? (Nx + 2 <= 128) : (M <= 128);
    if (wgrad3_ok(M, Nx)) {
        const int total_steps = n_evals * ((Bpad + 31) / 32);
        static const int target_chunks = getenv("RNDE_WGRAD3_CHUNKS") ? atoi(getenv("RNDE_WGRAD3_CHUNKS")) : 128;
        int sc = std::max(1, std::min({max_chunks > 0 ? max_chunks : target_chunks, total_steps, 256}));
        const int steps_per_chunk = (total_steps + sc - 1) / sc;
        sc = (total_steps + steps_per_chunk - 1) / steps_per_chunk;
        if ((size_t)(*chunk_cursor + sc) * (size_t)len > h->bw.slab_floats) { h->err = "weight-gradient slab overflow"; return RNDE_ERR_BAD_ARG; }
        const bool x3_off = getenv("RNDE_X3_WGRAD_OFF") != nullptr;
        const bool x3_half = getenv("RNDE_X3_WGRAD_HALF") != nullptr;
        const int TT4 = ((tall ? M : Nx + 2) + 15) / 16;
        if (h->x3_packed && !x3_off && !x3_half && TT4 >= 28 && TT4 <= 52) {
            static const int target4 = getenv("RNDE_WGRAD4_CHUNKS") ? atoi(getenv("RNDE_WGRAD4_CHUNKS")) : 64;
            int sc4 = std::max(1, std::min({max_chunks > 0 ? max_chunks / 2 : target4, total_steps, 256}));
            const int spc4 = (total_steps + sc4 - 1) / sc4;
            sc4 = (total_steps + spc4 - 1) / spc4;
            if ((size_t)(*chunk_cursor + sc4) * (size_t)len > h->bw.slab_floats) { h->err = "weight-gradient slab overflow"; return RNDE_ERR_BAD_ARG; }
            static constexpr decltype(&rnde_wgrad4x_kernel<true, 0>) kern4[2][2] = {{rnde_wgrad4x_kernel<false, 0>, rnde_wgrad4x_kernel<false, 1>},
                                                                                    {rnde_wgrad4x_kernel<true, 0>, rnde_wgrad4x_kernel<true, 1>}};
            static constexpr size_t lds4[2] = {kWx4LdsBytes, kWx4fLdsBytes};
            static DeviceOnce attr4;
            if (attr4.need()) {
                for (int t = 0; t < 2; ++t)
                    for (int f = 0; f < 2; ++f) HIPCHK(h, hipFuncSetAttribute((const void*)kern4[t][f], hipFuncAttributeMaxDynamicSharedMemorySize, (int)lds4[f]));
                attr4.done();
            }
            const dim3 g4(32 * ((sc4 + 7) / 8));
#if RNDE_WX4_ABL == 7 || RNDE_WX4_ABL == 8
            const bool q0 = true;
#else
            const char* ef = getenv("RNDE_X3_WGRAD_FEED");
            const bool q0 = getenv("RNDE_X3_WGRAD_Q0") != nullptr || (ef ? ef[0] == '0' : kWx4DefaultFeed == 0);
#endif
            const int feed = q0 ? 0 : 1;
            hipLaunchKernelGGL(kern4[tall][feed], g4, dim3(448), lds4[feed], s, ev, n_evals, spc4, sc4, M, Nx, Bpad, dst);
            HIPCHK(h, hipGetLastError());
            *chunk_cursor += sc4;
            return RNDE_OK;
        }
        static constexpr WgradKern kern3[2][2] = {{rnde_wgrad3_kernel<false>, rnde_wgrad3_kernel<true>}, {rnde_wgrad3x_kernel<false>, rnde_wgrad3x_kernel<true>}};
        static constexpr size_t lds3[2] = {(size_t)2 * 32 * (464 + 144) * sizeof(float) , kWxLdsBytes};
        static DeviceOnce attr3[2];
        const int x3 = (h->x3_packed && !x3_off) ? 1 : 0;
        if (attr3[x3].need()) {
            for (int t = 0; t < 2; ++t) HIPCHK(h, hipFuncSetAttribute((const void*)kern3[x3][t], hipFuncAttributeMaxDynamicSharedMemorySize, (int)lds3[x3]));
            attr3[x3].done();
        }
        hipLaunchKernelGGL(kern3[x3][tall], dim3(2, sc), dim3(448), lds3[x3], s, ev, n_evals, steps_per_chunk, M, Nx, Bpad, dst);
        HIPCHK(h, hipGetLastError());
        *chunk_cursor += sc;
        return RNDE_OK;
    }
    if (!legacy && fits) {
        const int pblocks = tall ? (M + 127) / 128 : (Nx + 2 + 127) / 128;
        const int total_steps = n_evals * ((Bpad + 31) / 32);
        static const int target_wgs = getenv("RNDE_WGRAD_WGS") ? atoi(getenv("RNDE_WGRAD_WGS")) : 768;
        int sc = std::max(1, std::min({target_wgs / pblocks, total_steps, 256}));
        const int steps_per_chunk = (total_steps + sc - 1) / sc;
        sc = (total_steps + steps_per_chunk - 1) / steps_per_chunk;
        if ((size_t)(*chunk_cursor + sc) * (size_t)len > h->bw.slab_floats) { h->err = "weight-gradient slab overflow"; return RNDE_ERR_BAD_ARG; }
        static constexpr WgradKern kern2[2] = {rnde_wgrad2_kernel<false>, rnde_wgrad2_kernel<true>};
        hipLaunchKernelGGL(kern2[tall], dim3(pblocks, sc), dim3(256), 0, s, ev, n_evals, steps_per_chunk, M, Nx, Bpad, dst);
        HIPCHK(h, hipGetLastError());
        *chunk_cursor += sc;
        return RNDE_OK;
    } else {
        if ((size_t)(*chunk_cursor + chunks) * (size_t)len > h->bw.slab_floats) { h->err = "weight-gradient slab overflow"; return RNDE_ERR_BAD_ARG; }
        static constexpr WgradKern kern[2] = {rnde_wgrad_kernel<4, 2>, rnde_wgrad_kernel<2, 4>};
        hipLaunchKernelGGL(kern[tall], dim3(blocks, chunks), dim3(64), 0, s, ev, n_evals, per_chunk, M, Nx, Bpad, dst);
    }
    HIPCHK(h, hipGetLastError());
    *chunk_cursor += chunks;
    return RNDE_OK;
}

static void gather_saveval_bar(rnde_node* h, const float* saveval_bar_host) {
    gather_svb(h->sv_index.data(), h->n_att, h->couple ? (float)h->couple_world : 1.f, saveval_bar_host, h->bw.h_svb);
}
static std::vector<SaveRange> save_ranges(const rnde_node* h) {
    std::vector<SaveRange> rng((size_t)std::max(1, h->n_att), SaveRange{0, 0});
    save_plan(h->saveat.data(), (int)h->saveat.size(), h->t0, h->h_meta, h->n_att, F_ACCEPT, rng.data());
    return rng;
}
static BwdParams fill_bwd_params(rnde_node* h, const float* u_bar_dev, float* x_bar_dev) {
    const BwdBuffers& b = h->bw;
    BwdParams Q{};
    Q.F = make_params(h, h->xcopy, h->B, h->t0, h->t1, 1);
    Q.U = b.U; Q.K1 = b.K1; Q.UB1 = b.UB1; Q.zi2 = b.zi2; Q.zi1 = b.zi1; Q.svb_att = b.svb_att;
    Q.bstate = b.bstate; Q.ibstate = b.ibstate; Q.bpart = b.bpart; Q.ipart = b.ipart;
    Q.ubar = u_bar_dev; Q.xbar = x_bar_dev; Q.tspan_out = b.tspan_out;
    Q.n_att = h->n_att; Q.track_ctrl = h->cfg.track_ctrl; Q.track_initdt = h->cfg.track_initdt; Q.reg_kind = h->cfg.regularize;
    Q.bpart_n = Q.F.nwg;
    Q.tspan_scale = h->couple ? 1.f / (float)h->couple_world : 1.f;
    Q.sv_T = (int)h->saveat.size();
    Q.sv_ubar0 = (!h->saveat.empty() && h->saveat[0] == h->t0) ? u_bar_dev : nullptr;
    return Q;
}
static rnde_status bwd_run(rnde_node* h, const float* u_bar_dev, const float* saveval_bar_host, float* x_bar_dev,
                           float* p_bar_dev, float* tspan_bar_host, hipStream_t s, bool sync, float* tspan_bar_dev) {
    HIPCHK(h, hipSetDevice(h->cfg.device));
    rnde_status st = bwd_prepare(h);
    if (st != RNDE_OK) return st;
    BwdBuffers& b = h->bw;
    int n_att = h->n_att;
    gather_saveval_bar(h, saveval_bar_host);
    const int ne_all = 2 + 6 * n_att;
    EvalDesc* const h_ev1 = b.h_ev1; EvalDesc* const h_ev2 = b.h_ev1 + ne_all; float* const h_svb_blob = (float*)(b.h_ev1 + 2 * (size_t)ne_all);
    EvalDesc* const d_ev1 = b.ev1;   EvalDesc* const d_ev2 = b.ev1 + ne_all;   float* const d_svb = (float*)(b.ev1 + 2 * (size_t)ne_all);
    memcpy(h_svb_blob, b.h_svb, (size_t)n_att * 4);
    BwdParams Q = fill_bwd_params(h, u_bar_dev, x_bar_dev);
    Q.svb_att = d_svb;
#ifdef RNDE_DIAG
    if (getenv("RNDE_DIAG_BWD")) { (void)h->diag_buf.reserve(2048); hipMemset(h->diag_buf, 0, 512); Q.F.dbg_out = h->diag_buf; }
#endif
    const long long A = (long long)h->D * Q.F.Bpad, HB = (long long)h->H * Q.F.Bpad;
    RecLayout L{A, HB};
    int ne = 2;
    h_ev2[0] = EvalDesc{b.zi2, h->h0, h->t0, 0};           h_ev1[0] = EvalDesc{b.zi1, h->xcopy, h->t0, 0};
    h_ev2[1] = EvalDesc{b.zi2 + A, h->h1, h->t0 + h->h_init->dt0, 0}; h_ev1[1] = EvalDesc{b.zi1 + HB, h->u1, h->t0 + h->h_init->dt0, 0};
    for (int n = 0; n < n_att; ++n) {
        const StepMeta& m = h->h_meta[n];
        const float* R = h->arena + (long long)m.rec * h->rec_stride;
        for (int sidx = 2; sidx <= 7; ++sidx) {
            const float ts = m.t + tsC(sidx - 1) * m.dt;
            h_ev2[ne] = EvalDesc{R + L.k(sidx), R + L.h(sidx), ts, 0};
            h_ev1[ne] = EvalDesc{R + L.z1(sidx), sidx < 7 ? R + L.g(sidx) : R + L.unew(), ts, 0};
            ++ne;
        }
    }
    HIPCHK(h, hipMemcpyAsync(b.ev1, b.h_ev1, 2 * (size_t)ne * sizeof(EvalDesc) + (size_t)n_att * 4, hipMemcpyHostToDevice, s));
    float* slab1 = b.slab;
    float* slab2w = b.slab + b.slab_floats;
    int cur1 = 0, cur2 = 0, evi = 0;
    const int per_chunk = std::max(1, (ne + 239) / 240);
    const int side_pct = h->wgrad_side_pct;
    const int sweep_cus = 8 * h->sR * ((Q.F.Bpad / 16 + 7) / 8);
    const bool side = h->persist == 1 && side_pct > 0 && n_att >= 8 && sweep_cus <= 224 &&
                      wgrad3_ok(h->H, h->D) && wgrad3_ok(h->D, h->H);
    const int side_att = side ? std::min(n_att, n_att * side_pct / 100) : 0;
    const int group = std::max(4, (side_att + 5) / 6);
    bool used_side = false;
    auto wgrad_group = [&](int lo, int hi, bool on_side) -> rnde_status {
        if (hi <= lo) return RNDE_OK;
        hipStream_t ws = s;
        if (on_side) {
            hipEvent_t ev = h->wevents[evi++ % 64];
            HIPCHK(h, hipEventRecord(ev, s));
            HIPCHK(h, hipStreamWaitEvent(h->wstream, ev, 0));
            ws = h->wstream; used_side = true;
        }
        rnde_status r = launch_wgrad_part(h, d_ev1 + lo, hi - lo, per_chunk, h->H, h->D, h->B, slab1, &cur1, ws, on_side ? 16 : 0);
        if (r != RNDE_OK) return r;
        return launch_wgrad_part(h, d_ev2 + lo, hi - lo, per_chunk, h->D, h->H, h->B, slab2w, &cur2, ws, on_side ? 16 : 0);
    };
    int hi_att = n_att;
    hipError_t e;
    h->tev_bwd = false;
    if (h->timing) HIPCHK(h, hipEventRecord(h->tev[2], s));
    {
        if (!h->rev_packed) {
            HIPCHK(h, stage_pack(h, h->pcopy, h->spwBt, 2, h->sMT, h->sKHb, s));
            HIPCHK(h, stage_pack(h, h->pcopy, h->spwDt, 3, h->sHT, h->sMT, s));
        }
        h->rev_packed = false;
        BStageParams BQ{};
        BQ.B = Q; BQ.p = h->pcopy; BQ.pwBt = h->spwBt; BQ.pwDt = h->spwDt; BQ.slab = h->slab2; BQ.x3Bt = h->x3Bt; BQ.x3Dt = h->x3Dt;
        BQ.UTB = b.UTB; BQ.UNB = b.UNB; BQ.UPB0 = b.UPB0; BQ.GB = b.GB;
        BQ.EXK = b.GB + 6 * A; BQ.EXG = b.GB + 7 * A; BQ.SVW = b.GB + 8 * A;
        BQ.sv_t = h->saveat.empty() ? nullptr : h->sv_t_dev; BQ.sv_ubar = u_bar_dev; BQ.nsave = (int)h->saveat.size();
        BQ.MT = h->sMT; BQ.WT = h->sWT; BQ.R = h->sR; BQ.C = Q.F.Bpad / 16; BQ.HT = h->sHT; BQ.KHb = h->sKHb;
        double* const bsum = (double*)(b.bstate + 2);
        const bool pre_reduce = h->persist == 1 && Q.bpart_n >= 896 && !getenv("RNDE_NO_BPART_REDUCE");
        if (pre_reduce) BQ.B.bsum = bsum;
        const dim3 grid(BQ.R * BQ.C), blk(64 * BQ.WT);
        const std::vector<SaveRange> rng = save_ranges(h);
        const int a2 = h->act2 ? 1 : 0;
        using BAttemptKern = decltype(&rnde_bstage_attempt_kernel<0, 0>);
        static constexpr BAttemptKern kAttempt[2][2] = {{rnde_bstage_attempt_kernel<0, 0>, rnde_bstage_attempt_kernel<0, 1>},
                                                        {rnde_bstage_attempt_kernel<1, 0>, rnde_bstage_attempt_kernel<1, 1>}};
        static constexpr BAttemptKern kAttemptX3[2][4] = {
            {rnde_bstage_attempt_kernel<0, 1, 1, 0>, rnde_bstage_attempt_kernel<0, 1, 1, 1>, rnde_bstage_attempt_kernel<0, 1, 1, 2>, rnde_bstage_attempt_kernel<0, 1, 1, 3>},
            {rnde_bstage_attempt_kernel<1, 1, 1, 0>, rnde_bstage_attempt_kernel<1, 1, 1, 1>, rnde_bstage_attempt_kernel<1, 1, 1, 2>, rnde_bstage_attempt_kernel<1, 1, 1, 3>}};
        static constexpr decltype(&rnde_bstage_kernel<0, BM_START>) kStage[2][2] = {{rnde_bstage_kernel<0, BM_START>, rnde_bstage_kernel<0, BM_STAGE>},
                                                                                   {rnde_bstage_kernel<1, BM_START>, rnde_bstage_kernel<1, BM_STAGE>}};
        static constexpr decltype(&rnde_binit_stage_kernel<0, 0>) kInit[2][4] = {
            {rnde_binit_stage_kernel<0, 0>, rnde_binit_stage_kernel<0, 1>, rnde_binit_stage_kernel<0, 2>, rnde_binit_stage_kernel<0, 3>},
            {rnde_binit_stage_kernel<1, 0>, rnde_binit_stage_kernel<1, 1>, rnde_binit_stage_kernel<1, 2>, rnde_binit_stage_kernel<1, 3>}};
        for (int n = n_att - 1; n >= 0; --n) {
            float c1 = 0.f, c2 = 0.f;
            eig_cotangent(h->cfg.regularize, b.h_svb[n], h->h_meta[n], &c1, &c2);
            const double qo = pow((double)h->h_meta[n].qold_in, (double)kBeta2);
            if (h->persist == 1) {
                PersistSync Y{h->tslab, h->pabort, h->pxcc, h->persist_spins};
                HIPCHK(h, slab_prepare(h, Q.F.Bpad, s));
                const dim3 pgrid(8 * BQ.R * ((BQ.C + 7) / 8));
                const bool fix = BQ.WT == 7 && BQ.HT == 7 && BQ.KHb == 7 && BQ.MT == 49 && BQ.R == 7 && h->D == 784 && h->H == 100 && !h->stage_generic;
                BAttemptKern kern = kAttempt[a2][fix];
                size_t lds = h->stage_lds;
                if (fix) {
                    lds = h->stage_lds + (size_t)(RNDE_BSTAGE_HDMA ? 1 : 0) * 6 * 7 * 2 * 1024;
                    static DeviceOnce attr;
                    if (attr.need()) {
                        for (int a = 0; a < 2; ++a) HIPCHK(h, hipFuncSetAttribute((const void*)kAttempt[a][1], hipFuncAttributeMaxDynamicSharedMemorySize, 160 * 1024));
                        attr.done();
                    }
                    const bool x3 = h->x3_packed && h->x3Bt && h->x3Dt && !getenv("RNDE_X3_REV_OFF");
                    if (x3) {
                        lds = sizeof(float) * ((size_t)2 * kX3ImageFloats + 64) + (size_t)(RNDE_BSTAGE_HDMA ? 1 : 0) * 6 * 7 * 2 * 1024;
                        static DeviceOnce attr3;
                        if (attr3.need()) {
                            for (int a = 0; a < 2; ++a)
                                for (int e = 0; e < 4; ++e) HIPCHK(h, hipFuncSetAttribute((const void*)kAttemptX3[a][e], hipFuncAttributeMaxDynamicSharedMemorySize, 160 * 1024));
                            attr3.done();
                        }
                        kern = kAttemptX3[a2][(h->saveat.empty() ? 0 : 1) | (h->cfg.regularize >= RNDE_REG_STIFF ? 2 : 0)];
                    }
                }
                hipLaunchKernelGGL(kern, pgrid, blk, lds, s, BQ, n, h->h_meta[n], c1, c2, rng[n].lo, rng[n].hi, Y, qo, b.h_svb[n]);
                if ((st = couple_sum(h, b.bpart + (size_t)(n & 1) * Q.bpart_n * 4, 4LL * Q.bpart_n, s)) != RNDE_OK) return st;
                if (pre_reduce && n > 0) hipLaunchKernelGGL(rnde_bpart_reduce_kernel, dim3(1), dim3(64), 0, s, Q, n, bsum);
                if (n >= n_att - side_att && (hi_att - n >= group || n == n_att - side_att)) {
                    st = wgrad_group(2 + 6 * n, 2 + 6 * hi_att, true);
                    if (st != RNDE_OK) return st;
                    hi_att = n;
                }
                continue;
            }
            hipLaunchKernelGGL(kStage[a2][BM_START], grid, blk, h->stage_lds, s, BQ, n, 0, h->h_meta[n], c1, c2, rng[n].lo, rng[n].hi, qo);
            for (int j = 6; j >= 1; --j) hipLaunchKernelGGL(kStage[a2][BM_STAGE], grid, blk, h->stage_lds, s, BQ, n, j, h->h_meta[n], c1, c2, rng[n].lo, rng[n].hi, qo);
            if ((st = couple_sum(h, b.bpart + (size_t)(n & 1) * Q.bpart_n * 4, 4LL * Q.bpart_n, s)) != RNDE_OK) return st;
        }
        HIPCHK(h, hipGetLastError());
        {
            for (int step = 0; step < 4; ++step) {
                hipLaunchKernelGGL(kInit[a2][step], grid, blk, h->stage_lds, s, BQ);
                if ((step & 1) && (st = couple_sum(h, Q.ipart + (step / 2) * 4LL * Q.F.nwg, 4LL * Q.F.nwg, s)) != RNDE_OK) return st;
            }
            hipLaunchKernelGGL(rnde_bfin_kernel, dim3(1), dim3(64), 0, s, Q);
            HIPCHK(h, hipGetLastError());
        }
    }
    if (h->timing) HIPCHK(h, hipEventRecord(h->tev[3], s));
    st = wgrad_group(0, 2 + 6 * hi_att, false);
    if (st != RNDE_OK) return st;
    if (used_side) {
        hipEvent_t ev = h->wevents[64];
        HIPCHK(h, hipEventRecord(ev, h->wstream));
        HIPCHK(h, hipStreamWaitEvent(s, ev, 0));
    }
    if (cur1 > 16 && cur2 > 16) {
        const long long len1 = (long long)h->H * (h->D + 2), len2 = (long long)h->D * (h->H + 2);
        const size_t seg_r = std::max((size_t)len1, (size_t)len2);
        float* r1 = b.slab_r; float* r2 = b.slab_r + 16 * seg_r;
        const int pg1 = (cur1 + 15) / 16, g1 = (cur1 + pg1 - 1) / pg1, pg2 = (cur2 + 15) / 16, g2 = (cur2 + pg2 - 1) / pg2;
        const int grid = (int)std::min<long long>((std::max(len1, len2) + 255) / 256, 2048);
        ReducePair A{{{slab1, r1, len1, cur1, pg1}, {slab2w, r2, len2, cur2, pg2}}};
        hipLaunchKernelGGL(rnde_wgrad_reduce_pair, dim3(grid, std::max(g1, g2), 2), dim3(256), 0, s, A);
        ReducePair Bp{{{r1, p_bar_dev, len1, g1, g1}, {r2, p_bar_dev + (size_t)h->H * (h->D + 2), len2, g2, g2}}};
        hipLaunchKernelGGL(rnde_wgrad_reduce_pair, dim3(grid, 1, 2), dim3(256), 0, s, Bp);
        HIPCHK(h, hipGetLastError());
    } else {
        HIPCHK(h, launch_wgrad_reduce(slab1, cur1, (long long)h->H * (h->D + 2), b.slab_r, p_bar_dev, s));
        HIPCHK(h, launch_wgrad_reduce(slab2w, cur2, (long long)h->D * (h->H + 2), b.slab_r, p_bar_dev + (size_t)h->H * (h->D + 2), s));
    }
    if (h->timing) { HIPCHK(h, hipEventRecord(h->tev[4], s)); h->tev_bwd = true; }
#ifdef RNDE_DIAG
    if (h->persist == 1 && getenv("RNDE_DIAG_BWD")) {
        unsigned long long hst[64] = {0};
        hipStreamSynchronize(s);
        hipMemcpy(hst, h->diag_buf, sizeof(hst), hipMemcpyDeviceToHost);
        fprintf(stderr, "persistent reverse attempt (workgroup 0 thread 0, cycles): START %lld (entry->weights issued %lld, ->w1t %lld, ->array loads issued %lld, finish_attempt_scalars %lld, scalar chain %lld, vector part %lld), its phase D + put %lld\n", (long long)(hst[1]-hst[0]), (long long)(hst[43]-hst[0]), (long long)(hst[44]-hst[43]), (long long)(hst[40]-hst[44]), (long long)(hst[41]-hst[40]), (long long)(hst[42]-hst[41]), (long long)(hst[1]-hst[42]), (long long)(hst[2]-hst[1]));
        for (int st = 0; st < 6; ++st) { const unsigned long long* q = hst + 3 + 5 * st; const unsigned long long prev = st == 0 ? hst[2] : hst[7 + 5 * (st - 1)];
            fprintf(stderr, "  stage j=%d: poll %lld A %lld B %lld C %lld D+put %lld\n", 6 - st, (long long)(q[0]-prev), (long long)(q[1]-q[0]), (long long)(q[2]-q[1]), (long long)(q[3]-q[2]), st < 5 ? (long long)(q[4]-q[3]) : 0LL); }
        fprintf(stderr, "  total %lld cycles to the end of stage 1, END (reduction of the 21 partial sums) %lld; in START's vector part the wait for the record's k arrays %lld\n",
                (long long)(hst[34]-hst[0]), (long long)(hst[35]-hst[34]), (long long)(hst[45]-hst[42]));
    }
#endif
    if (!sync) {
        if (tspan_bar_dev) HIPCHK(h, hipMemcpyAsync(tspan_bar_dev, b.tspan_out, 8, hipMemcpyDeviceToDevice, s));
        h->have_tape = false;
        h->pending_bwd = h->persist == 1;
        return RNDE_OK;
    }
    HIPCHK(h, hipMemcpyAsync(h->h_scal, b.tspan_out, 8, hipMemcpyDeviceToHost, s));
    persist_check_enqueue(h, h->sR * (Q.F.Bpad / 16), s);
    HIPCHK(h, hipStreamSynchronize(s));
    if (h->couple && rnde_comm_health(h->couple) != RNDE_OK) { h->err = std::string("coupled controller: ") + rnde_comm_last_error(h->couple); return RNDE_ERR_HIP; }
    if (tspan_bar_host) { tspan_bar_host[0] = h->h_scal[0]; tspan_bar_host[1] = h->h_scal[1]; }
    h->have_tape = false;
    if (persist_check_result(h, Q.F.Bpad / 16, h->sR, s)) {
        h->err = "persistent reverse kernel abandoned its hand-off (tape consumed): rerun forward + backward, the multi-launch kernels are now in use";
        return RNDE_ERR_HIP;
    }
    return RNDE_OK;
}

static rnde_status head_reserve(rnde_node* h, int32_t B, int32_t n_classes) {
    const size_t need = (size_t)B * n_classes + B + (size_t)kHeadChunks * n_classes * h->D;
    HIPCHK(h, h->head_ws.reserve(need));
    return RNDE_OK;
}
extern "C" rnde_status rnde_classifier_head(rnde_node* h, const float* u_dev, const float* p3_dev, const float* y_dev,
                                            int32_t B, int32_t n_classes, float* logits_out_dev, float* u_bar_dev,
                                            float* p3_bar_dev, float* ce_out_dev, void* stream) {
    if (!h || B < 1 || n_classes < 1 || n_classes > kHeadMaxC) return RNDE_ERR_BAD_ARG;
    hipStream_t s = (hipStream_t)stream;
    const rnde_status rs = head_reserve(h, B, n_classes);
    if (rs != RNDE_OK) return rs;
    float* delta = h->head_ws;
    float* ce_col = h->head_ws + (size_t)B * n_classes;
    if (h->D > 256 * kHeadRowsPerThread) { h->err = "classifier head: D <= 1024"; return RNDE_ERR_BAD_ARG; }
    if (n_classes == 10) hipLaunchKernelGGL((rnde_head_col_kernel<10>), dim3(B), dim3(256), 0, s, u_dev, p3_dev, y_dev, h->D, n_classes, B,
                       logits_out_dev, u_bar_dev, delta, ce_col);
    else hipLaunchKernelGGL((rnde_head_col_kernel<0>), dim3(B), dim3(256), 0, s, u_dev, p3_dev, y_dev, h->D, n_classes, B,
                       logits_out_dev, u_bar_dev, delta, ce_col);
    float* partial = ce_col + B;
    hipLaunchKernelGGL(rnde_head_wgrad_kernel, dim3((h->D + 255) / 256, kHeadChunks), dim3(256), 0, s, u_dev, (const float*)delta,
                       h->D, n_classes, B, partial);
    hipLaunchKernelGGL(rnde_head_reduce_kernel, dim3((n_classes * h->D + 255) / 256), dim3(256), 0, s, (const float*)partial,
                       (const float*)delta, (const float*)ce_col, h->D, n_classes, B, p3_bar_dev, ce_out_dev);
    HIPCHK(h, hipGetLastError());
    return RNDE_OK;
}

extern "C" rnde_status rnde_node_classifier_grad(rnde_node* h, const float* x_dev, const float* p2_dev, const float* p3_dev,
                                                 const float* y_dev, int32_t B, int32_t n_classes, float t0, float t1,
                                                 float lambda, float* p2_bar_dev, float* p3_bar_dev, float* x_bar_dev,
                                                 float* ce_out_dev, float* reg_out_host, int64_t* nfe_out, rnde_comm* comm,
                                                 void* stream) {
    if (!h || !x_dev || !p2_dev || !p3_dev || !y_dev || !p2_bar_dev || !p3_bar_dev || !ce_out_dev) return RNDE_ERR_BAD_ARG;
    RNDE_TILED_REFUSE(h, "rnde_node_classifier_grad is not served (the fused training step runs on the stage engine: two-layer dynamics, rnde_node_create with col_tile 0)");
    if (h->engine != 2) { h->err = "rnde_node_classifier_grad: two-layer dynamics on the stage engine (col_tile 0)"; return RNDE_ERR_BAD_ARG; }
    if (B < 1 || B > h->cfg.max_batch) { h->err = "bad B or tspan"; return RNDE_ERR_BAD_ARG; }
    HIPCHK(h, hipSetDevice(h->cfg.device));
    const size_t A = (size_t)h->D * B;
    HIPCHK(h, h->cg_ws.reserve(3 * A));
    HIPCHK(h, h->ev_host.create(hipEventDisableTiming));
    if (n_classes < 1 || n_classes > kHeadMaxC) return RNDE_ERR_BAD_ARG;
    rnde_status st = head_reserve(h, B, n_classes);
    if (st != RNDE_OK) return st;
    float* u = h->cg_ws; float* ubar = h->cg_ws + A; float* xbar = x_bar_dev ? x_bar_dev : h->cg_ws + 2 * A;
    h->cg_sv.resize((size_t)h->cfg.max_attempts + 1);
// ... 229 lines not shown
```

### regneuralde.jl_amd/csrc/rnde_stage.h

```cpp
#pragma once
#include "rnde_fwd.h"

namespace rnde {

constexpr int kSCB = 16;
constexpr int kSMaxW = 8;
constexpr int kSMaxHT = 8;

struct StageParams {
    StepParams F;
    const float* p;
    const f32x4* pwB;
    const f32x4* pwD;
    float* slab;
    int MT, WT, R, C, HT, K2b;
    int Bpad16;
};

__device__ __forceinline__ int kperm(int k) { return (k & ~15) | ((k & 3) << 2) | ((k >> 2) & 3); }

__device__ __forceinline__ f32x4 mfma16(float a, float b, f32x4 c) {
    return __builtin_amdgcn_mfma_f32_16x16x4f32(a, b, c, 0, 0, 0);
}
__device__ __forceinline__ float add_square_unfused(float acc, float d) {
#pragma clang fp contract(off)
    const float m = d * d;
    return acc + m;
}
__device__ __forceinline__ f32x4 fma4(float s, f32x4 a, f32x4 c) { return __builtin_elementwise_fma((f32x4){s, s, s, s}, a, c); }

__device__ __forceinline__ f32x4 stage_pack_elem(const float* __restrict__ p, int which, int D, int H, int Kb, long long i) {
    const float* W1 = p;
    const float* b1 = W1 + (size_t)H * (D + 1);
    const float* W2 = b1 + H;
    const float* b2 = W2 + (size_t)D * (H + 1);
    const int l = (int)(i & 63);
    const int kb = (int)((i >> 6) % Kb);
    const int T = (int)((i >> 6) / Kb);
    const int m = 16 * T + (l & 15);
    f32x4 v;
#pragma unroll
    for (int q = 0; q < 4; ++q) {
        const int k = 16 * kb + 4 * q + (l >> 4);
        float w = 0.f;
        if (which == 0) { if (m < D) w = k <= H ? W2[(size_t)k * D + m] : (k == H + 1 ? b2[m] : 0.f); }
        else if (which == 1) { if (m < H && k < D) w = W1[(size_t)k * H + m]; }
        else if (which == 2) { if (m < D && k < H) w = W1[(size_t)m * H + k]; }
        else { if (m <= H && k < D) w = W2[(size_t)m * D + k]; }
        v[q] = w;
    }
    return v;
}
static __global__ void rnde_stage_pack_kernel(const float* __restrict__ p, f32x4* __restrict__ dst, int which, int D, int H,
                                       int MTrows, int Kb) {
    const long long total = (long long)MTrows * Kb * 64;
    for (long long i = blockIdx.x * (long long)blockDim.x + threadIdx.x; i < total; i += (long long)gridDim.x * blockDim.x)
        dst[i] = stage_pack_elem(p, which, D, H, Kb, i);
}

struct PackJob { void* dst; const float* src; long long total; int kind, which, kdim, pad; };
struct PackJobs { PackJob j[8]; };
static __global__ void rnde_pack_all_kernel(const float* __restrict__ p, const PackJobs J, int D, int H) {
    const PackJob job = J.j[blockIdx.y];
    for (long long i = blockIdx.x * (long long)blockDim.x + threadIdx.x; i < job.total; i += (long long)gridDim.x * blockDim.x) {
        if (job.kind == 0) ((f32x4*)job.dst)[i] = stage_pack_elem(p, job.which, D, H, job.kdim, i);
        else if (job.kind == 2) ((float*)job.dst)[i] = (job.src ? job.src : p)[i];
        else ((f32x4*)job.dst)[i] = ((const f32x4*)(job.src ? job.src : p))[i];
    }
}

__device__ __forceinline__ void dense_points(const StepParams& P, const RecLayout& L, const float* Rp, float tp, float dtp_, float tnew,
                                             int lo, int hi, size_t co, int gcol, int r0, bool colok, bool vec) {
    const f32x4 up = ld_tile(Rp + L.upc() + co, r0, P.D, true, vec);
    f32x4 k[7];
    k[0] = ld_tile(Rp + L.k1c() + co, r0, P.D, true, vec);
#pragma unroll
    for (int j = 1; j < 7; ++j) k[j] = ld_tile(Rp + L.k(j + 1) + co, r0, P.D, true, vec);
    const f32x4 un = ld_tile(Rp + L.unew() + co, r0, P.D, true, vec);
    for (int idx = lo; idx < hi; ++idx) {
        const float ts = P.sv_t[idx];
        f32x4 o = un;
        if (ts != tnew) {
            float b[7];
            dense_weights((ts - tp) / dtp_, b);
            f32x4 acc = b[0] * k[0];
#pragma unroll
            for (int j = 1; j < 7; ++j) acc += b[j] * k[j];
            o = up + dtp_ * acc;
        }
        st_tile(P.sv_out + ((size_t)gcol * P.nsave + idx) * P.D, r0, P.D, colok, vec && ((P.D & 3) == 0), o);
    }
}

enum { SM_START = 0, SM_STAGE = 1, SM_LAST = 2, SM_I1 = 3, SM_I2 = 4, SM_I3 = 5, SM_I4 = 6, SM_FEVAL1 = 7, SM_FEVAL2 = 8 };

__device__ __forceinline__ f32x4 ld4(const float* colbase, int r0, int D, bool ok, bool vec) { return ld_tile(colbase, r0, D, ok, vec); }
__device__ __forceinline__ void st4(float* colbase, int r0, int D, bool ok, bool vec, f32x4 v) { st_tile(colbase, r0, D, ok, vec, v); }

__device__ __forceinline__ void init_norm_parts_u0_f0(const StepParams& P, const f32x4& xv, const f32x4& kv, int r0, bool colok, float& part0, float& part1) {
    if (colok) {
#pragma unroll
        for (int i = 0; i < 4; ++i) {
            if (r0 + i < P.D) {
                const float sk = P.abstol + fabsf(xv[i]) * P.reltol;
                const float a = xv[i] / sk, b = kv[i] / sk;
                part0 += a * a; part1 += b * b;
            }
        }
    }
}
__device__ __forceinline__ float init_dt0_rule(const StepParams& P, double s0, double s1, bool writer, float* d1_out = nullptr) {
    const double N = (double)P.D * (double)P.Bn;
    const float d0 = (float)sqrt(s0 / N), d1 = (float)sqrt(s1 / N), dtmax = P.t1 - P.t0;
    float dt0;
    int c0 = 0, cl = 0;
    if (d0 < 1e-5f || d1 < 1e-5f) { dt0 = 1e-6f; c0 = 1; } else dt0 = (d0 / d1) / 100.f;
    if (dtmax < dt0) { dt0 = dtmax; cl = 1; }
    if (writer) { P.initrec->d0 = d0; P.initrec->d1 = d1; P.initrec->dt0 = dt0; P.initrec->dt0_const = c0; P.initrec->dt0_clamped = cl; }
    if (d1_out) *d1_out = d1;
    return dt0;
}
__device__ __forceinline__ f32x4 init_euler_step(const f32x4& xv, float dt0, const f32x4& f0) { return xv + dt0 * f0; }
__device__ __forceinline__ void init_norm_part_df(const StepParams& P, const f32x4& xv, const f32x4& f0, const f32x4& kv, int r0, bool colok, float& part0) {
    if (colok) {
#pragma unroll
        for (int i = 0; i < 4; ++i) {
            if (r0 + i < P.D) {
                const float sk = P.abstol + fabsf(xv[i]) * P.reltol;
                const float a = (kv[i] - f0[i]) / sk;
                part0 += a * a;
            }
        }
    }
}

template <int ACT2, int MODE>
__global__ __launch_bounds__(64 * kSMaxW) void rnde_stage_kernel(const StageParams Q, const int n, const int s) {
    const StepParams& P = Q.F;
    extern __shared__ __attribute__((aligned(16))) float smem[];
    const int KH = 16 * Q.K2b + 4, KG = 16 * Q.WT + 4;
    float* HL = smem;
    float* GL = HL + kSCB * KH;
    float* RED = GL + kSCB * KG;
    const int tid = threadIdx.x, lane = tid & 63;
    const int w = __builtin_amdgcn_readfirstlane(tid >> 6);
    const int rb = blockIdx.x / Q.C, ct = blockIdx.x - rb * Q.C;
    const int col = lane & 15, gcol = ct * kSCB + col;
    const bool colok = gcol < P.B;
// ... 356 lines not shown
```

### regneuralde.jl_amd/csrc/rnde_wgradx.h

```cpp
#pragma once
#include "rnde_x3.h"

namespace rnde {

constexpr int kWxRowShorts = 40;
constexpr int kWxTallRows = 400, kWxNarrowRows = 112;
constexpr int kWxPlaneShortsT = kWxTallRows * kWxRowShorts, kWxPlaneShortsS = kWxNarrowRows * kWxRowShorts;
constexpr size_t kWxLdsBytes = (size_t)3 * (kWxPlaneShortsT + kWxPlaneShortsS) * 2;

template <bool TALL_IS_Z>
__global__ __launch_bounds__(448) void rnde_wgrad3x_kernel(const EvalDesc* __restrict__ evals, int n_evals, int per_chunk, int M, int Nx, int Bpad, float* __restrict__ slab) {
    constexpr int KC = 32;
    extern __shared__ __attribute__((aligned(16))) unsigned short wxs[];
    unsigned short* TP = wxs;
    unsigned short* SP = wxs + 3 * kWxPlaneShortsT;
    const int tid = threadIdx.x, lane = tid & 63, w = __builtin_amdgcn_readfirstlane(tid >> 6);
    const int mrow = lane & 15, kk = lane >> 4;
    const int TR = TALL_IS_Z ? M : Nx + 2, SR = TALL_IS_Z ? Nx + 2 : M;
    const int TRp = TALL_IS_Z ? M : Nx, SRp = TALL_IS_Z ? Nx : M;
    const int TT = (TR + 15) >> 4, T0 = (TT + 1) >> 1;
    const int half = blockIdx.x, chunk = blockIdx.y;
    const int tile_lo = half ? T0 : 0, tile_hi = half ? TT : T0, ntile = tile_hi - tile_lo;
    const int row_lo = 16 * tile_lo, nrow = 16 * ntile;
    const int steps_per_eval = (Bpad + KC - 1) / KC;
// ... 50 lines not shown
    auto spill = [&]() {
#pragma unroll
        for (int jj = 0; jj < 5; ++jj) {
            const int kind = u_kind[jj];
            if (kind == 0) continue;
            const int o8 = u_dst[jj] % kWxRowShorts;
            float v[8];
#pragma unroll
            for (int j = 0; j < 8; ++j) v[j] = kind == 1 ? stg[jj][j] : ((kind == 2 || kind == 3) && o8 + j < stg_ncols ? (kind == 2 ? stg_t : 1.f) : 0.f);
            unsigned hi[4], mid[4], lo[4];
#pragma unroll
            for (int j = 0; j < 4; ++j) x3_split2(v[2 * j], v[2 * j + 1], hi[j], mid[j], lo[j]);
            unsigned short* d = wxs + u_dst[jj];
            const int ps = jj < 4 ? kWxPlaneShortsT : kWxPlaneShortsS;
            *(x3u4*)d = (x3u4){hi[0], hi[1], hi[2], hi[3]};
            *(x3u4*)(d + ps) = (x3u4){mid[0], mid[1], mid[2], mid[3]};
            *(x3u4*)(d + 2 * ps) = (x3u4){lo[0], lo[1], lo[2], lo[3]};
        }
    };
    auto fragT = [&](int tile, int pl) { return *(const x3u4*)(TP + pl * kWxPlaneShortsT + (16 * tile + mrow) * kWxRowShorts + 8 * kk); };
    auto fragS = [&](int tile, int pl) { return *(const x3u4*)(SP + pl * kWxPlaneShortsS + (16 * tile + mrow) * kWxRowShorts + 8 * kk); };

    if (total_steps > 0) { fetch(); spill(); }
    __syncthreads();
    for (int step = 0; step < total_steps; ++step) {
        if (step + 1 < total_steps) fetch();
#pragma unroll
        for (int ps = 0; ps < 2; ++ps) {
            x3u4 a[2][3];
#pragma unroll
            for (int i = 0; i < 2; ++i) {
                const int ii = 2 * ps + i, tile = (ii < 3 || has3) ? w + 7 * ii : w;
#pragma unroll
                for (int pl = 0; pl < 3; ++pl) a[i][pl] = fragT(tile, pl);
            }
#pragma unroll
            for (int n = 0; n < 7; ++n) {
                __builtin_amdgcn_sched_barrier(0);
                const x3u4 bh = fragS(n, 0), bm = fragS(n, 1), bl = fragS(n, 2);
#define WX_TERM(PA, BV) _Pragma("unroll") for (int i = 0; i < 2; ++i) if (2 * ps + i < 3 || has3) acc[2 * ps + i][n] = x3_mfma(a[i][PA], BV, acc[2 * ps + i][n]);
                WX_TERM(2, bh) WX_TERM(0, bl) WX_TERM(1, bm) WX_TERM(1, bh) WX_TERM(0, bm) WX_TERM(0, bh)
#undef WX_TERM
            }
        }
        __syncthreads();
        if (step + 1 < total_steps) spill();
        __syncthreads();
    }
    float* out = slab + (size_t)chunk * M * (Nx + 2);
#pragma unroll
    for (int i = 0; i < 4; ++i) {
        if (w + 7 * i < ntile) {
#pragma unroll
            for (int n = 0; n < 7; ++n) {
                const int sr = 16 * n + mrow;
#pragma unroll
                for (int q = 0; q < 4; ++q) {
                    const int tr = row_lo + 16 * (w + 7 * i) + 4 * kk + q;
                    if (tr < TR && sr < SR) out[TALL_IS_Z ? (size_t)sr * M + tr : (size_t)tr * M + sr] = acc[i][n][q];
                }
            }
        }
    }
}

#ifndef RNDE_WX4_SB
#define RNDE_WX4_SB 1
#endif
#ifndef RNDE_WX4_ABL
#define RNDE_WX4_ABL 0
#endif
constexpr int kWx4TallRows = 208;
constexpr int kWx4PlaneT = kWx4TallRows * kWxRowShorts, kWx4PlaneS = kWxNarrowRows * kWxRowShorts;
constexpr int kWx4ImageShorts = 3 * (kWx4PlaneT + kWx4PlaneS);
constexpr size_t kWx4LdsBytes = (size_t)2 * kWx4ImageShorts * 2;
constexpr int kWx4fRowShorts = 32;
constexpr int kWx4fWideShorts = (kWx4TallRows + 4) * kWx4fRowShorts;
constexpr int kWx4fPlane = (kWx4TallRows + 4 + kWxNarrowRows + 4) * kWx4fRowShorts;
constexpr int kWx4fImageShorts = 3 * kWx4fPlane;
constexpr size_t kWx4fLdsBytes = (size_t)2 * kWx4fImageShorts * 2;
constexpr int kWx4DefaultFeed = 1;

template <bool TALL_IS_Z, int FEED>
__global__ __launch_bounds__(448) void rnde_wgrad4x_kernel(const EvalDesc* __restrict__ evals, int n_evals, int per_chunk, int n_chunks, int M, int Nx, int Bpad,
                                                           float* __restrict__ slab) {
    constexpr int KC = 32;
    extern __shared__ __attribute__((aligned(16))) unsigned short wxs[];
    const int tid = threadIdx.x, lane = tid & 63, w = __builtin_amdgcn_readfirstlane(tid >> 6);
    const int mrow = lane & 15, kk = lane >> 4;
    const int lin = blockIdx.x, xcd = lin & 7, within = lin >> 3;
    const int chunk = (within >> 2) * 8 + xcd, part = within & 3;
    if (chunk >= n_chunks) return;
    const int TR = TALL_IS_Z ? M : Nx + 2, SR = TALL_IS_Z ? Nx + 2 : M;
    const int TRp = TALL_IS_Z ? M : Nx, SRp = TALL_IS_Z ? Nx : M;
    const int TT = (TR + 15) >> 4, base = TT >> 2, rem = TT & 3;
    const int ntile = base + (part < rem ? 1 : 0), tile_lo = part * base + (part < rem ? part : rem);
    const int row_lo = 16 * tile_lo, nrow = 16 * ntile;
    const int steps_per_eval = (Bpad + KC - 1) / KC;
    const int s_lo = chunk * per_chunk, s_hi = min(n_evals * steps_per_eval, s_lo + per_chunk);
    const int total_steps = max(0, s_hi - s_lo);
    x3f4 acc[2][7];
#pragma unroll
    for (int i = 0; i < 2; ++i)
#pragma unroll
        for (int n = 0; n < 7; ++n) acc[i][n] = (x3f4){0.f, 0.f, 0.f, 0.f};
    const bool has2 = w + 7 < ntile;
    const int tile1 = has2 ? w + 7 : w;

    constexpr unsigned kNoSrc = 0x7FFFFF00u;
    const bool wide_wave = w < 4;
    const int Rp = wide_wave ? TRp : SRp;
    const int nunit = wide_wave ? nrow : kWxNarrowRows;
    const int ut = wide_wave ? tid : tid - 256;
    const int nquad = nunit >> 2;
    const bool u_real = ut < nunit;
    const int uid = ut % nunit;
    const int uq = FEED ? uid % nquad : uid >> 2, uo = FEED ? uid / nquad : uid & 3;
#if RNDE_WX4_ABL == 7
    const int lq = uid % nquad, lo8 = uid / nquad;
#else
    const int lq = uq, lo8 = uo;
#endif
    const int u_gr = (wide_wave ? row_lo : 0) + 4 * lq;
#if RNDE_WX4_ABL == 8
    const bool u_mem = u_gr < Rp && u_real;
#else
    const bool u_mem = u_gr < Rp && (FEED == 0 || u_real);
#endif
    const bool u_syn = u_gr == Rp && (wide_wave ? !TALL_IS_Z : TALL_IS_Z);
    const float syn_f = u_syn ? 1.f : 0.f;
    const unsigned u_voff = u_mem ? 4u * (unsigned)(u_gr + 8 * lo8 * Rp) : kNoSrc;
#if RNDE_WX4_ABL == 8
    const int u_dst = (wide_wave ? 0 : 3 * kWx4PlaneT) + 4 * uq * kWxRowShorts + (u_real ? 8 * uo : 32);
#else
    const int u_dst = (wide_wave ? 0 : 3 * kWx4PlaneT) + 4 * uq * kWxRowShorts + 8 * uo;
#endif
    const int u_ps = wide_wave ? kWx4PlaneT : kWx4PlaneS;
    int f_dst[4] = {0, 0, 0, 0};
    int f_frag[2] = {0, 0};
    if (FEED) {
        const int qa = u_real ? uq & 3 : lane & 3, qt = u_real ? (uq >> 2) & 1 : (lane >> 2) & 1, qo = u_real ? uo : 0;
        const int line = (wide_wave ? 0 : kWx4fWideShorts) + 128 * (u_real ? uq : wide_wave ? kWx4TallRows / 4 : kWxNarrowRows / 4);
#pragma unroll
        for (int b = 0; b < 4; ++b) f_dst[b] = line + 32 * ((b + qa) & 3) + 8 * ((qo ^ (4 - qa) ^ qt) & 3);
        const int fa = mrow >> 2;
        f_frag[0] = 128 * fa + 32 * ((mrow + fa) & 3) + 8 * ((kk ^ (4 - fa)) & 3);
        f_frag[1] = f_frag[0] ^ 8;
    }
    const int f_a0 = f_frag[w & 1] + 512 * w, f_a1 = f_frag[tile1 & 1] + 512 * tile1;
    int e_nx = s_lo / steps_per_eval, cs_nx = s_lo - e_nx * steps_per_eval, left = total_steps;
    x3f4 stg[2][8];
    float stg_t[2] = {0.f, 0.f}; int stg_ncols[2] = {0, 0};
    auto fetch = [&](auto set_c) {
        constexpr int SET = decltype(set_c)::value;
        const int e = e_nx, c0 = cs_nx * KC;
        {
            const bool adv = --left > 0, wrap = cs_nx + 1 == steps_per_eval;
            e_nx = (adv && wrap) ? e_nx + 1 : e_nx;
            cs_nx = adv ? (wrap ? 0 : cs_nx + 1) : cs_nx;
        }
        stg_t[SET] = evals[e].t;
        stg_ncols[SET] = min(KC, Bpad - c0);
        const float* src = wide_wave == TALL_IS_Z ? evals[e].Z : evals[e].X;
        __amdgpu_buffer_rsrc_t rs = __builtin_amdgcn_make_buffer_rsrc((void*)src, 0, 4 * Rp * Bpad, 0x00020000);
#pragma unroll
        for (int j = 0; j < 8; ++j)
            stg[SET][j] = __builtin_bit_cast(x3f4, __builtin_amdgcn_raw_buffer_load_b128(rs, (int)u_voff, 4 * (c0 + j) * Rp, 0));
    };
    unsigned abl_sink = 0u;
    auto spill_row = [&](unsigned short* img, int i, auto set_c) {
        constexpr int SET = decltype(set_c)::value;
        float v[8];
#pragma unroll
// ... 15 lines not shown
        *(x3u4*)d = (x3u4){hi[0], hi[1], hi[2], hi[3]};
        *(x3u4*)(d + ps) = (x3u4){mid[0], mid[1], mid[2], mid[3]};
        *(x3u4*)(d + 2 * ps) = (x3u4){lo[0], lo[1], lo[2], lo[3]};
#endif
    };
    unsigned short* const img0 = wxs;
    unsigned short* const img1 = wxs + (FEED ? kWx4fImageShorts : kWx4ImageShorts);
    if (total_steps == 0) return;
    typedef std::integral_constant<int, 0> S0;
    typedef std::integral_constant<int, 1> S1;
    fetch(S0{});
#pragma unroll
    for (int i = 0; i < 4; ++i) spill_row(img0, i, S0{});
    fetch(S0{});
    fetch(S1{});
    __syncthreads();
    auto one_step = [&](const unsigned short* cur, unsigned short* nxt, auto more_c, auto set_c) {
        constexpr bool MORE = decltype(more_c)::value;
        const unsigned short* SPc = cur + (FEED ? kWx4fWideShorts : 3 * kWx4PlaneT);
        auto fragT = [&](int i, int pl) {
            if (FEED) return *(const x3u4*)(cur + pl * kWx4fPlane + (i ? f_a1 : f_a0));
            return *(const x3u4*)(cur + pl * kWx4PlaneT + (16 * (i ? tile1 : w) + mrow) * kWxRowShorts + 8 * kk);
        };
        auto fragS = [&](int tile, int pl) {
            if (FEED) return *(const x3u4*)(SPc + pl * kWx4fPlane + f_frag[tile & 1] + 512 * tile);
            return *(const x3u4*)(SPc + pl * kWx4PlaneS + (16 * tile + mrow) * kWxRowShorts + 8 * kk);
        };
        x3u4 a[2][3];
#pragma unroll
        for (int pl = 0; pl < 3; ++pl) { a[0][pl] = fragT(0, pl); a[1][pl] = fragT(1, pl); }
        x3u4 bh = fragS(0, 0), bm = fragS(0, 1), bl = fragS(0, 2);
#pragma unroll
        for (int n = 0; n < 7; ++n) {
            x3u4 nh = bh, nm = bm, nl = bl;
#if RNDE_WX4_ABL != 3 && RNDE_WX4_ABL != 4
            if (n < 6) { nh = fragS(n + 1, 0); nm = fragS(n + 1, 1); nl = fragS(n + 1, 2); }
#endif
#if RNDE_WX4_ABL != 1 && RNDE_WX4_ABL != 2 && RNDE_WX4_ABL != 4
            if (MORE && n < 4) spill_row(nxt, n, set_c);
#endif
#if RNDE_WX4_ABL != 2 && RNDE_WX4_ABL != 4
            if (MORE && n == 4) fetch(set_c);
#endif
#define WX4_TERM(PA, BV) { acc[0][n] = x3_mfma(a[0][PA], BV, acc[0][n]); acc[1][n] = x3_mfma(a[1][PA], BV, acc[1][n]); }
            WX4_TERM(2, bh) WX4_TERM(0, bl) WX4_TERM(1, bm) WX4_TERM(1, bh) WX4_TERM(0, bm) WX4_TERM(0, bh)
#undef WX4_TERM
            bh = nh; bm = nm; bl = nl;
#if RNDE_WX4_SB
            __builtin_amdgcn_sched_barrier(0);
#endif
        }
    };
    int step = 0;
    for (; step + 2 < total_steps; step += 2) {
        one_step(img0, img1, std::true_type{}, S0{});
        __syncthreads();
        one_step(img1, img0, std::true_type{}, S1{});
        __syncthreads();
    }
    if (total_steps - step == 2) {
        one_step(img0, img1, std::true_type{}, S0{});
        __syncthreads();
        one_step(img1, nullptr, std::false_type{}, S1{});
    } else one_step(img0, nullptr, std::false_type{}, S0{});
#if RNDE_WX4_ABL == 5
    if (abl_sink == 0x12345678u) slab[0] = 1.f;
#endif
    float* out = slab + (size_t)chunk * M * (Nx + 2);
#pragma unroll
    for (int i = 0; i < 2; ++i) {
        if (w + 7 * i < ntile) {
#pragma unroll
            for (int n = 0; n < 7; ++n) {
                const int sr = 16 * n + mrow;
#pragma unroll
                for (int q = 0; q < 4; ++q) {
                    const int tr = row_lo + 16 * (w + 7 * i) + 4 * kk + q;
                    if (tr < TR && sr < SR) out[TALL_IS_Z ? (size_t)sr * M + tr : (size_t)tr * M + sr] = acc[i][n][q];
                }
            }
        }
    }
}

}
```

### regneuralde.jl_amd/csrc/rnde_x3.h

```cpp
#pragma once
#include <hip/hip_runtime.h>

namespace rnde {

typedef unsigned x3u4 __attribute__((ext_vector_type(4)));
typedef unsigned x3u2 __attribute__((ext_vector_type(2)));
typedef __bf16 x3bf8 __attribute__((ext_vector_type(8)));
typedef float x3f4 __attribute__((ext_vector_type(4)));

constexpr int kX3K = 136;
constexpr int kX3PlaneShorts = 16 * kX3K;
constexpr int kX3ImageFloats = 3 * kX3PlaneShorts / 2;

__device__ __forceinline__ unsigned x3_cvt2(float a, float b) {
    unsigned r;
    asm("v_cvt_pk_bf16_f32 %0, %1, %2" : "=v"(r) : "v"(a), "v"(b));
    return r;
}
#ifndef RNDE_X3_DOT2
#define RNDE_X3_DOT2 0
#endif
typedef __bf16 x3bf2 __attribute__((ext_vector_type(2)));
typedef float x3f2 __attribute__((ext_vector_type(2)));
__device__ __forceinline__ void x3_split2(float x0, float x1, unsigned& hi, unsigned& mid, unsigned& lo) {
#pragma clang fp contract(off)
#if RNDE_X3_DOT2
    unsigned kl = 0x0000BF80u, kh = 0xBF800000u;
    asm("" : "+s"(kl));
    asm("" : "+s"(kh));
    const x3bf2 bl = __builtin_bit_cast(x3bf2, kl), bh = __builtin_bit_cast(x3bf2, kh);
    const x3bf2 h = __builtin_convertvector((x3f2){x0, x1}, x3bf2);
    const float r0 = __builtin_amdgcn_fdot2_f32_bf16(h, bl, x0, false), r1 = __builtin_amdgcn_fdot2_f32_bf16(h, bh, x1, false);
    const x3bf2 m = __builtin_convertvector((x3f2){r0, r1}, x3bf2);
    const float s0 = __builtin_amdgcn_fdot2_f32_bf16(m, bl, r0, false), s1 = __builtin_amdgcn_fdot2_f32_bf16(m, bh, r1, false);
    hi = __builtin_bit_cast(unsigned, h);
    mid = __builtin_bit_cast(unsigned, m);
    lo = __builtin_bit_cast(unsigned, __builtin_convertvector((x3f2){s0, s1}, x3bf2));
#else
    hi = x3_cvt2(x0, x1);
    const float r0 = x0 - __uint_as_float(hi << 16), r1 = x1 - __uint_as_float(hi & 0xFFFF0000u);
    mid = x3_cvt2(r0, r1);
    const float s0 = r0 - __uint_as_float(mid << 16), s1 = r1 - __uint_as_float(mid & 0xFFFF0000u);
    lo = x3_cvt2(s0, s1);
#endif
}
__device__ __forceinline__ void x3_store4(unsigned short* img, int col, int k0, const x3f4& v) {
    unsigned h01, m01, l01, h23, m23, l23;
    x3_split2(v[0], v[1], h01, m01, l01);
    x3_split2(v[2], v[3], h23, m23, l23);
    unsigned short* p = img + col * kX3K + k0;
    *(x3u2*)p = (x3u2){h01, h23};
    *(x3u2*)(p + kX3PlaneShorts) = (x3u2){m01, m23};
    *(x3u2*)(p + 2 * kX3PlaneShorts) = (x3u2){l01, l23};
}
__device__ __forceinline__ x3u4 x3_frag(const unsigned short* img, int pl, int s, int lane) {
    return *(const x3u4*)(img + pl * kX3PlaneShorts + (lane & 15) * kX3K + 32 * s + 8 * (lane >> 4));
}
__device__ __forceinline__ x3f4 x3_mfma(const x3u4& a, const x3u4& b, const x3f4& c) {
    return __builtin_amdgcn_mfma_f32_16x16x32_bf16(__builtin_bit_cast(x3bf8, a), __builtin_bit_cast(x3bf8, b), c, 0, 0, 0);
}
template <int NS>
__device__ __forceinline__ x3f4 x3_tile(const x3u4 (&wa)[NS][3], const unsigned short* img, int lane) {
    x3f4 aL = {0.f, 0.f, 0.f, 0.f}, aN = {0.f, 0.f, 0.f, 0.f}, aM = {0.f, 0.f, 0.f, 0.f}, aH = {0.f, 0.f, 0.f, 0.f};
    x3u4 bh = x3_frag(img, 0, 0, lane), bm = x3_frag(img, 1, 0, lane), bl = x3_frag(img, 2, 0, lane);
#pragma unroll
    for (int s = 0; s < NS; ++s) {
        x3u4 nh = bh, nm = bm, nl = bl;
        if (s + 1 < NS) { nh = x3_frag(img, 0, s + 1, lane); nm = x3_frag(img, 1, s + 1, lane); nl = x3_frag(img, 2, s + 1, lane); }
        __builtin_amdgcn_sched_barrier(0);
        aL = x3_mfma(wa[s][2], bh, aL);
        aM = x3_mfma(wa[s][1], bh, aM);
        aH = x3_mfma(wa[s][0], bh, aH);
        aN = x3_mfma(wa[s][1], bm, aN);
        aL = x3_mfma(wa[s][0], bl, aL);
        aM = x3_mfma(wa[s][0], bm, aM);
        __builtin_amdgcn_sched_barrier(0);
        bh = nh; bm = nm; bl = nl;
    }
    return ((aL + aN) + aM) + aH;
}

struct X3PackDst { x3u4* d[4]; };
static __global__ void rnde_x3_pack_kernel(const float* __restrict__ p, const X3PackDst dst, int D, int H, int MT, int WT, int R, int HT) {
    const float* W1 = p;
    const float* b1 = W1 + (size_t)H * (D + 1);
    const float* W2 = b1 + H;
    const float* b2 = W2 + (size_t)D * (H + 1);
    const long long nB = (long long)MT * 4 * 64, nD = (long long)HT * R * 4 * 64, per = nB + nD;
    const int nimg = dst.d[2] ? 2 : 1;
    for (long long i = blockIdx.x * (long long)blockDim.x + threadIdx.x; i < nimg * per; i += (long long)gridDim.x * blockDim.x) {
        const int rev = (int)(i / per);
        const long long ii = i - rev * per;
        const bool isD = ii >= nB;
        const long long q = isD ? ii - nB : ii;
        const int l = (int)(q & 63), s = (int)((q >> 6) & 3), tile = (int)(q >> 8);
        float wv[8];
#pragma unroll
        for (int j = 0; j < 8; ++j) {
            const int k = 32 * s + 8 * (l >> 4) + j;
            float w = 0.f;
            if (!isD) {
                const int m = 16 * tile + (l & 15);
                if (m < D) {
                    if (!rev) w = k <= H ? W2[(size_t)k * D + m] : (k == H + 1 ? b2[m] : 0.f);
                    else if (k < H) w = W1[(size_t)m * H + k];
                }
            } else {
                const int wt = tile / R, rb = tile % R;
                const int m = 16 * wt + (l & 15), row = 16 * WT * rb + k;
                if (k < 16 * WT && row < D) {
                    if (!rev) { if (m < H) w = W1[(size_t)row * H + m]; }
                    else if (m <= H) w = W2[(size_t)m * D + row];
                }
            }
            wv[j] = w;
        }
        unsigned hi[4], mid[4], lo[4];
#pragma unroll
        for (int j = 0; j < 4; ++j) x3_split2(wv[2 * j], wv[2 * j + 1], hi[j], mid[j], lo[j]);
        x3u4* o = dst.d[2 * rev + (isD ? 1 : 0)] + ((size_t)(tile * 4 + s) * 3) * 64 + l;
        o[0] = (x3u4){hi[0], hi[1], hi[2], hi[3]};
        o[64] = (x3u4){mid[0], mid[1], mid[2], mid[3]};
        o[128] = (x3u4){lo[0], lo[1], lo[2], lo[3]};
    }
}

}
```

Baseline: 314,900 samples/s.

## Fold reverse-tail kernels: pair binit stages, single-pass wgrad reduce, paired wgrad4x launch

Several reverse-pass tail launches are merged to cut kernel-launch and global-memory round-trip overhead. The four binit stage kernels become two pair kernels that hand partial sums over a persistent slab with polling, and the two-level wgrad reduction collapses into one fold kernel. The two wgrad4x launches are combined into one paired kernel, and the x3 bf16 weight pack is folded into the pack_all kernel behind an opt-in environment switch. The pair kernels depend on co-residency and spin-sync, which adds a risk of stalls, and the fold reduce changes summation order.

```diff
diff --git a/include/rnde.h b/include/rnde.h
--- a/include/rnde.h
+++ b/include/rnde.h
@@ -127,6 +127,7 @@
 int32_t     rnde_node_fallback_count(const rnde_node* h);
 int32_t     rnde_node_launches_per_attempt(const rnde_node* h);
 int32_t     rnde_node_one_launch_solves(const rnde_node* h);
+void        rnde_node_tail_folds(const rnde_node* h, int64_t counts[4]);
 #define RNDE_MATRIX_F32 0
 #define RNDE_MATRIX_BF16X3 1
 rnde_status rnde_node_set_matrix_mode(rnde_node* h, int32_t mode);
diff --git a/regneuralde.jl_amd/_lib.py b/regneuralde.jl_amd/_lib.py
--- a/regneuralde.jl_amd/_lib.py
+++ b/regneuralde.jl_amd/_lib.py
@@ -232,7 +232,7 @@
            "rnde_node_forward", "rnde_node_forward_saveat", "rnde_node_forward_everystep", "rnde_node_forward_replay", "rnde_node_backward", "rnde_node_backward_async", "rnde_node_release_tape", "rnde_node_forward_host",
            "rnde_node_backward_host", "rnde_node_steps", "rnde_debug_feval", "rnde_debug_attempt",
            "rnde_bench_attempt", "rnde_bench_attempt_taped", "rnde_bench_attempt_cold_tape", "rnde_node_set_timing", "rnde_node_timing", "rnde_node_last_attempts", "rnde_node_fallback_count",
-           "rnde_node_launches_per_attempt", "rnde_node_one_launch_solves", "rnde_node_set_matrix_mode", "rnde_node_matrix_mode", "rnde_classifier_head", "rnde_node_classifier_grad", "rnde_momentum_step", "rnde_momentum_step_scaled", "rnde_adam_step",
+           "rnde_node_launches_per_attempt", "rnde_node_one_launch_solves", "rnde_node_tail_folds", "rnde_node_set_matrix_mode", "rnde_node_matrix_mode", "rnde_classifier_head", "rnde_node_classifier_grad", "rnde_momentum_step", "rnde_momentum_step_scaled", "rnde_adam_step",
            "rnde_comm_unique_id", "rnde_comm_create", "rnde_comm_destroy", "rnde_comm_world", "rnde_comm_last_error", "rnde_comm_library", "rnde_comm_allreduce", "rnde_comm_create_local_group", "rnde_comm_health", "rnde_comm_window_create", "rnde_comm_window_destroy", "rnde_comm_create_peers", "rnde_comm_path", "rnde_node_set_coupling", "rnde_tapes_create", "rnde_tapes_destroy", "rnde_tapes_last_error", "rnde_tapes_in_use", "rnde_tapes_node", "rnde_tapes_forward", "rnde_tapes_backward", "rnde_tapes_release",
            "rnde_nsde_param_count", "rnde_nsde_create", "rnde_nsde_destroy", "rnde_nsde_last_error", "rnde_nsde_forward",
            "rnde_nsde_forward_saveat", "rnde_nsde_forward_everystep", "rnde_nsde_forward_replay", "rnde_nsde_backward", "rnde_nsde_backward_async", "rnde_nsde_classifier_head", "rnde_nsde_classifier_grad", "rnde_nsde_steps", "rnde_nsde_debug_attempt", "rnde_nsde_set_pre_act", "rnde_nsde_moment_grad", "rnde_moment_loss", "rnde_adabelief_step", "rnde_nsde_timing", "rnde_normal_fill", "rnde_latent_create", "rnde_latent_destroy", "rnde_latent_last_error", "rnde_latent_param_counts", "rnde_latent_encode",
diff --git a/regneuralde.jl_amd/csrc/rnde.hip b/regneuralde.jl_amd/csrc/rnde.hip
--- a/regneuralde.jl_amd/csrc/rnde.hip
+++ b/regneuralde.jl_amd/csrc/rnde.hip
@@ -462,12 +462,20 @@
     };
     add_copy(h->pcopy, nullptr, (long long)h->P);
     if (x_src) add_copy(h->xcopy, x_src, x_floats);
+    const bool x3_in = h->x3 && h->x3B && h->x3D && h->persist == 1 && !h->stage_generic && tail_switch("RNDE_X3_PACK_FOLD", false);
+    if (x3_in) {
+        const bool rev = h->x3Bt && h->x3Dt;
+        J.x3 = X3PackDst{{(x3u4*)h->x3B.get(), (x3u4*)h->x3D.get(), rev ? (x3u4*)h->x3Bt.get() : nullptr, rev ? (x3u4*)h->x3Dt.get() : nullptr}};
+        J.MT = h->sMT; J.WT = h->sWT; J.R = h->sR; J.HT = h->sHT;
+        add(nullptr, x3_pack_count(J.x3, J.MT, J.R, J.HT), 4, 0, 0);
+    }
     long long most = 0;
     for (int i = 0; i < n; ++i) most = std::max(most, J.j[i].total);
     const int grid = (int)std::min<long long>((most + 255) / 256, 256);
     hipLaunchKernelGGL(rnde_pack_all_kernel, dim3(grid, n), dim3(256), 0, s, p_dev, J, h->D, h->H);
     HIPCHK(h, hipGetLastError());
     h->rev_packed = true;
+    if (x3_in) { h->x3_fwd = true; h->x3_packed = true; ++h->tail_folds[2]; return RNDE_OK; }
     return x3_pack(h, p_dev, true, s);
 }
 hipError_t slab_prepare(rnde_node* h, int Bpad, hipStream_t s) {
@@ -1001,6 +1009,7 @@
 extern "C" int32_t rnde_node_fallback_count(const rnde_node* h) { return h ? h->persist_fallbacks : 0; }
 
 extern "C" int32_t rnde_node_one_launch_solves(const rnde_node* h) { return h ? h->one_launch_solves : 0; }
+extern "C" void rnde_node_tail_folds(const rnde_node* h, int64_t counts[4]) { for (int i = 0; i < 4; ++i) counts[i] = h ? (int64_t)h->tail_folds[i] : 0; }
 extern "C" rnde_status rnde_node_set_matrix_mode(rnde_node* h, int32_t mode) {
     if (!h) return RNDE_ERR_BAD_ARG;
     if (mode != RNDE_MATRIX_F32 && mode != RNDE_MATRIX_BF16X3) { h->err = "matrix mode: 0 (fp32-input MFMA) or 1 (bf16x3 on the matrix cores)"; return RNDE_ERR_BAD_ARG; }
diff --git a/regneuralde.jl_amd/csrc/rnde_binit_stage.h b/regneuralde.jl_amd/csrc/rnde_binit_stage.h
--- a/regneuralde.jl_amd/csrc/rnde_binit_stage.h
+++ b/regneuralde.jl_amd/csrc/rnde_binit_stage.h
@@ -1,40 +1,61 @@
 #pragma once
 #include "rnde_bstage.h"
+#include "rnde_stage_persist.h"
 
 namespace rnde {
 
-template <int ACT2, int STEP>
-__global__ __launch_bounds__(64 * kSMaxW) void rnde_binit_stage_kernel(const BStageParams Q) {
+struct BinitGeo {
+    int tid, lane, w, rb, ct, wg, col, gcol, T, r0, KZ, KG;
+    bool colok, vec, writer, tile_ok;
+    long long A, HB;
+    size_t co;
+    float *ZL, *GL, *RED;
+};
+__device__ __forceinline__ BinitGeo binit_geo(const BStageParams& Q, float* smem, int rb, int ct) {
+    const StepParams& P = Q.B.F;
+    BinitGeo g;
+    g.KZ = 16 * Q.KHb + 4; g.KG = 16 * Q.WT + 4;
+    g.ZL = smem;
+    g.GL = g.ZL + kSCB * g.KZ;
+    g.RED = g.GL + kSCB * g.KG;
+    g.tid = threadIdx.x; g.lane = g.tid & 63;
+    g.w = __builtin_amdgcn_readfirstlane(g.tid >> 6);
+    g.rb = rb; g.ct = ct; g.wg = rb * Q.C + ct;
+    g.col = g.lane & 15; g.gcol = ct * kSCB + g.col;
+    g.colok = g.gcol < P.B;
+    g.vec = (P.D & 3) == 0;
+    g.writer = (g.wg == 0 && g.tid == 0);
+    g.T = rb * Q.WT + g.w;
+    g.r0 = 16 * g.T + 4 * (g.lane >> 4);
+    g.tile_ok = g.T < Q.MT;
+    g.A = (long long)P.D * P.Bpad; g.HB = (long long)P.H * P.Bpad;
+    g.co = (size_t)g.gcol * P.D;
+    return g;
+}
+__device__ __forceinline__ constexpr int binit_pair_buf(int phase) { return phase == 1 ? 1 : 0; }
+__device__ __forceinline__ constexpr int binit_pair_clear(int phase) { return phase == 1 ? 0 : 1; }
+
+__device__ __forceinline__ void binit_load_wB(const BStageParams& Q, const BinitGeo& g, f32x4 (&wB)[kSMaxHT]) {
+#pragma unroll
+    for (int kb = 0; kb < kSMaxHT; ++kb)
+        if (kb < Q.KHb && g.tile_ok) wB[kb] = Q.pwBt[((size_t)g.T * Q.KHb + kb) * 64 + g.lane];
+}
+
+template <int ACT2, int kPhase, bool PAIR>
+__device__ __forceinline__ void binit_phase_d(const BStageParams& Q, const PersistSync& Y, const BinitGeo& g, f32x4& f0v_out) {
 #pragma clang fp contract(off)
     const BwdParams& Bq = Q.B;
     const StepParams& P = Bq.F;
-    extern __shared__ __attribute__((aligned(16))) float smem[];
-    const int KZ = 16 * Q.KHb + 4, KG = 16 * Q.WT + 4;
-    float* ZL = smem;
-    float* GL = ZL + kSCB * KZ;
-    float* RED = GL + kSCB * KG;
-    const int tid = threadIdx.x, lane = tid & 63;
-    const int w = __builtin_amdgcn_readfirstlane(tid >> 6);
-    const int rb = blockIdx.x / Q.C, ct = blockIdx.x - rb * Q.C;
-    const int wg = blockIdx.x;
-    const int col = lane & 15, gcol = ct * kSCB + col;
-    const bool colok = gcol < P.B;
-    const bool vec = (P.D & 3) == 0;
-    const bool writer = (blockIdx.x == 0 && tid == 0);
-    const int T = rb * Q.WT + w;
-    const int r0 = 16 * T + 4 * (lane >> 4);
-    const bool tile_ok = T < Q.MT;
-    const long long A = (long long)P.D * P.Bpad, HB = (long long)P.H * P.Bpad;
-    const size_t co = (size_t)gcol * P.D;
+    const int lane = g.lane, w = g.w, rb = g.rb, ct = g.ct, col = g.col, gcol = g.gcol, r0 = g.r0, KG = g.KG;
+    const bool colok = g.colok, vec = g.vec, writer = g.writer, tile_ok = g.tile_ok;
+    const long long A = g.A;
+    const size_t co = g.co;
+    float* GL = g.GL;
     const double N = (double)P.D * (double)P.Bn;
     const InitRec ir = *P.initrec;
     const float dt0 = ir.dt0;
-    constexpr bool kD = (STEP == 0 || STEP == 2);
-    constexpr int kPhase = STEP < 2 ? 1 : 2;
-    constexpr int par = STEP < 2 ? 0 : 1;
-
-    float dot = 0.f, tau = 0.f;
-    if constexpr (kD) {
+    constexpr int par = kPhase == 1 ? 0 : 1;
+    {
         f32x4 wD[kSMaxW];
 #pragma unroll
         for (int kb = 0; kb < kSMaxW; ++kb)
@@ -50,6 +71,7 @@
                 K1v = ld4(Bq.K1 + co, r0, P.D, true, vec);
             }
         }
+        f0v_out = f0v;
         f32x4 v = {0.f, 0.f, 0.f, 0.f};
         if constexpr (kPhase == 1) {
             double tb, dtpb, qoldb, t1b, t0b;
@@ -112,6 +134,7 @@
         for (int i = 0; i < 4; ++i) GL[col * KG + kperm(16 * w + 4 * (lane >> 4) + i)] = tile_ok ? v[i] : 0.f;
         __syncthreads();
         f32x4* sl = (f32x4*)Q.slab + ((((size_t)par * Q.C + ct) * Q.R + rb) * Q.HT) * 64;
+        const size_t tile0 = (((size_t)binit_pair_buf(kPhase) * Q.C + ct) * Q.R + rb) * Q.HT;
         const float* gbp = GL + col * KG + 4 * (lane >> 4);
         f32x4 bg[kSMaxW];
 #pragma unroll
@@ -127,7 +150,8 @@
                     acc1 = mfma16(wD[kb][3], bg[kb][3], acc1);
                 }
             }
-            sl[(size_t)w * 64 + lane] = acc0 + acc1;
+            if constexpr (PAIR) slab_put(Y.tslab, tile0 + w, lane, acc0 + acc1);
+            else sl[(size_t)w * 64 + lane] = acc0 + acc1;
         }
         for (int ht = w + Q.WT; ht < Q.HT; ht += Q.WT) {
             f32x4 acc0 = {0.f, 0.f, 0.f, 0.f}, acc1 = {0.f, 0.f, 0.f, 0.f};
@@ -141,23 +165,37 @@
                     acc1 = mfma16(a[3], bg[kb][3], acc1);
                 }
             }
-            sl[(size_t)ht * 64 + lane] = acc0 + acc1;
-        }
-        return;
-    } else {
-        f32x4 wB[kSMaxHT];
-#pragma unroll
-        for (int kb = 0; kb < kSMaxHT; ++kb)
-            if (kb < Q.KHb && tile_ok) wB[kb] = Q.pwBt[((size_t)T * Q.KHb + kb) * 64 + lane];
+            if constexpr (PAIR) slab_put(Y.tslab, tile0 + ht, lane, acc0 + acc1);
+            else sl[(size_t)ht * 64 + lane] = acc0 + acc1;
+        }
+    }
+}
+
+template <int ACT2, int kPhase, bool PAIR>
+__device__ __forceinline__ void binit_phase_ab(const BStageParams& Q, const PersistSync& Y, const BinitGeo& g, const f32x4 (&wB)[kSMaxHT], const f32x4& f0v) {
+#pragma clang fp contract(off)
+    const BwdParams& Bq = Q.B;
+    const StepParams& P = Bq.F;
+    const int tid = g.tid, lane = g.lane, w = g.w, rb = g.rb, ct = g.ct, wg = g.wg, col = g.col, gcol = g.gcol, r0 = g.r0, KZ = g.KZ;
+    const bool colok = g.colok, vec = g.vec, tile_ok = g.tile_ok;
+    const long long HB = g.HB;
+    const size_t co = g.co;
+    float* ZL = g.ZL; float* RED = g.RED;
+    constexpr int par = kPhase == 1 ? 0 : 1;
+    float dot = 0.f, tau = 0.f;
+    {
         const float* hsrc = kPhase == 1 ? P.h1 : P.h0;
         float* z1dst = kPhase == 1 ? Bq.zi1 + HB : Bq.zi1;
         const float* W1t = Q.p + (size_t)P.H * P.D;
         const f32x4* sl = (const f32x4*)Q.slab + (((size_t)par * Q.C + ct) * Q.R) * Q.HT * 64;
-        f32x4 f0v = {0.f, 0.f, 0.f, 0.f};
-        if (kPhase == 1 && tile_ok) f0v = ld4(P.f0 + co, r0, P.D, true, vec);
+        const size_t tclr0 = (((size_t)binit_pair_clear(kPhase) * Q.C + ct) * Q.R + rb) * Q.HT;
         for (int ht = w; ht < Q.HT; ht += Q.WT) {
             f32x4 z = {0.f, 0.f, 0.f, 0.f};
-            for (int r = 0; r < Q.R; ++r) z += sl[((size_t)r * Q.HT + ht) * 64 + lane];
+            if constexpr (PAIR) {
+                if (slab_poll_sum(Y, binit_pair_buf(kPhase), Q.C, Q.R, Q.HT, ct, ht, lane, z)) slab_clear(Y.tslab, tclr0 + ht, lane);
+            } else {
+                for (int r = 0; r < Q.R; ++r) z += sl[((size_t)r * Q.HT + ht) * 64 + lane];
+            }
             const int h0 = 16 * ht + 4 * (lane >> 4);
 #pragma unroll
             for (int i = 0; i < 4; ++i) {
@@ -222,4 +260,37 @@
     }
 }
 
-}
+template <int ACT2, int STEP>
+__global__ __launch_bounds__(64 * kSMaxW) void rnde_binit_stage_kernel(const BStageParams Q) {
+    extern __shared__ __attribute__((aligned(16))) float smem[];
+    const int rb = blockIdx.x / Q.C, ct = blockIdx.x - rb * Q.C;
+    const BinitGeo g = binit_geo(Q, smem, rb, ct);
+    constexpr int kPhase = STEP < 2 ? 1 : 2;
+    const PersistSync none{};
+    f32x4 f0v = {0.f, 0.f, 0.f, 0.f};
+    if constexpr (STEP == 0 || STEP == 2) {
+        binit_phase_d<ACT2, kPhase, false>(Q, none, g, f0v);
+    } else {
+        const StepParams& P = Q.B.F;
+        f32x4 wB[kSMaxHT];
+        binit_load_wB(Q, g, wB);
+        if (kPhase == 1 && g.tile_ok) f0v = ld4(P.f0 + g.co, g.r0, P.D, true, g.vec);
+        binit_phase_ab<ACT2, kPhase, false>(Q, none, g, wB, f0v);
+    }
+}
+
+template <int ACT2, int PHASE>
+__global__ __launch_bounds__(64 * kSMaxW) void rnde_binit_pair_kernel(const BStageParams Q, const PersistSync Y) {
+    extern __shared__ __attribute__((aligned(16))) float smem[];
+    const int rb = (blockIdx.x >> 3) % Q.R, ct = 8 * ((blockIdx.x >> 3) / Q.R) + (blockIdx.x & 7);
+    if (ct >= Q.C) return;
+    const BinitGeo g = binit_geo(Q, smem, rb, ct);
+    if (g.tid == 0) Y.xcc[g.wg] = __builtin_amdgcn_s_getreg((3 << 11) | (0 << 6) | 20) & 15;
+    f32x4 wB[kSMaxHT];
+    binit_load_wB(Q, g, wB);
+    f32x4 f0v;
+    binit_phase_d<ACT2, PHASE, true>(Q, Y, g, f0v);
+    binit_phase_ab<ACT2, PHASE, true>(Q, Y, g, wB, f0v);
+}
+
+}
diff --git a/regneuralde.jl_amd/csrc/rnde_bwd.h b/regneuralde.jl_amd/csrc/rnde_bwd.h
--- a/regneuralde.jl_amd/csrc/rnde_bwd.h
+++ b/regneuralde.jl_amd/csrc/rnde_bwd.h
@@ -459,5 +459,34 @@
         o[i] = s;
     }
 }
-
-}
+static __global__ void rnde_wgrad_reduce_fold_pair(const ReducePair R) {
+    const ReduceJob J = R.j[blockIdx.z];
+    const int pg = J.per_group, groups = (J.n_chunks + pg - 1) / pg;
+    for (long long i = blockIdx.x * (long long)blockDim.x + threadIdx.x; i < J.len; i += (long long)gridDim.x * blockDim.x) {
+        float s[16];
+#pragma unroll
+        for (int g = 0; g < 16; ++g) s[g] = 0.f;
+        for (int k = 0; k < pg; k += 2) {
+            float v[2][16];
+#pragma unroll
+            for (int u = 0; u < 2; ++u)
+#pragma unroll
+                for (int g = 0; g < 16; ++g) {
+                    const int c = g * pg + k + u;
+                    const bool ok = k + u < pg && c < J.n_chunks;
+                    const float x = __builtin_nontemporal_load(J.slab + (size_t)(ok ? c : 0) * J.len + i);
+                    v[u][g] = ok ? x : 0.f;
+                }
+#pragma unroll
+            for (int u = 0; u < 2; ++u)
+#pragma unroll
+                for (int g = 0; g < 16; ++g) s[g] += v[u][g];
+        }
+        float total = 0.f;
+#pragma unroll
+        for (int g = 0; g < 16; ++g) total = g < groups ? total + s[g] : total;
+        J.out[i] = total;
+    }
+}
+
+}
diff --git a/regneuralde.jl_amd/csrc/rnde_node.h b/regneuralde.jl_amd/csrc/rnde_node.h
--- a/regneuralde.jl_amd/csrc/rnde_node.h
+++ b/regneuralde.jl_amd/csrc/rnde_node.h
@@ -72,6 +72,7 @@
     int persist_clean = 0, persist_retry_after = 8, persist_fallbacks = 0;
     int persist2 = -1;
     int persist = 0, persist_spins = kPersistMaxSpins; int tslab_Bpad = -1; size_t tslab_bytes = 0; DevBuf<float> tslab; unsigned *pabort = nullptr, *pxcc = nullptr; unsigned* h_pchk = nullptr;
+    long long tail_folds[4] = {0, 0, 0, 0};
     int stage_solve = 1; MeetRes s_meet; int one_launch_solves = 0;
     int x3 = 0; DevBuf<unsigned char> x3B, x3D, x3Bt, x3Dt; bool x3_packed = false, x3_fwd = false;
     DevBuf<float> f0, h0, u1, f1, h1, arena;
@@ -158,6 +159,7 @@
 }
 
 static const rnde_status RNDE_INTERNAL_RETRY = static_cast<rnde_status>(100);
+static inline bool tail_switch(const char* name, bool by_default = true) { const char* e = getenv(name); return e ? e[0] != '0' : by_default; }
 StepParams make_params(rnde_node* h, const float* x, int B, float t0, float t1, int tape);
 MwParams make_mw_params(rnde_node* h, const StepParams& P);
 ChainParams make_chain_params(rnde_node* h, const StepParams& P);
diff --git a/regneuralde.jl_amd/csrc/rnde_reverse.hip b/regneuralde.jl_amd/csrc/rnde_reverse.hip
--- a/regneuralde.jl_amd/csrc/rnde_reverse.hip
+++ b/regneuralde.jl_amd/csrc/rnde_reverse.hip
@@ -74,6 +74,29 @@
     return getenv("RNDE_WGRAD_LEGACY") == nullptr && getenv("RNDE_WGRAD_V2") == nullptr && M % 4 == 0 && Nx % 4 == 0 && wide > 656 &&
            wide <= 800 && narrow <= 112;
 }
+struct Wx4Plan { bool ok; int spc4, sc4, feed; };
+static Wx4Plan wgrad4_plan(const rnde_node* h, int n_evals, int M, int Nx, int Bpad, int max_chunks) {
+    Wx4Plan q{false, 0, 0, 0};
+    if (n_evals <= 0 || !wgrad3_ok(M, Nx)) return q;
+    const bool tall = M >= Nx;
+    const int total_steps = n_evals * ((Bpad + 31) / 32);
+    const bool x3_off = getenv("RNDE_X3_WGRAD_OFF") != nullptr;
+    const bool x3_half = getenv("RNDE_X3_WGRAD_HALF") != nullptr;
+    const int TT4 = ((tall ? M : Nx + 2) + 15) / 16;
+    if (!(h->x3_packed && !x3_off && !x3_half && TT4 >= 28 && TT4 <= 52)) return q;
+    static const int target4 = getenv("RNDE_WGRAD4_CHUNKS") ? atoi(getenv("RNDE_WGRAD4_CHUNKS")) : 64;
+    int sc4 = std::max(1, std::min({max_chunks > 0 ? max_chunks / 2 : target4, total_steps, 256}));
+    const int spc4 = (total_steps + sc4 - 1) / sc4;
+    sc4 = (total_steps + spc4 - 1) / spc4;
+#if RNDE_WX4_ABL == 7 || RNDE_WX4_ABL == 8
+    const bool q0 = true;
+#else
+    const char* ef = getenv("RNDE_X3_WGRAD_FEED");
+    const bool q0 = getenv("RNDE_X3_WGRAD_Q0") != nullptr || (ef ? ef[0] == '0' : kWx4DefaultFeed == 0);
+#endif
+    q.ok = true; q.spc4 = spc4; q.sc4 = sc4; q.feed = q0 ? 0 : 1;
+    return q;
+}
 using WgradKern = decltype(&rnde_wgrad3_kernel<true>);
 static rnde_status launch_wgrad_part(rnde_node* h, const EvalDesc* ev, int n_evals, int per_chunk, int M, int Nx, int Bpad,
                                      float* slab, int* chunk_cursor, hipStream_t s, int max_chunks = 0) {
@@ -95,13 +118,9 @@
         sc = (total_steps + steps_per_chunk - 1) / steps_per_chunk;
         if ((size_t)(*chunk_cursor + sc) * (size_t)len > h->bw.slab_floats) { h->err = "weight-gradient slab overflow"; return RNDE_ERR_BAD_ARG; }
         const bool x3_off = getenv("RNDE_X3_WGRAD_OFF") != nullptr;
-        const bool x3_half = getenv("RNDE_X3_WGRAD_HALF") != nullptr;
-        const int TT4 = ((tall ? M : Nx + 2) + 15) / 16;
-        if (h->x3_packed && !x3_off && !x3_half && TT4 >= 28 && TT4 <= 52) {
-            static const int target4 = getenv("RNDE_WGRAD4_CHUNKS") ? atoi(getenv("RNDE_WGRAD4_CHUNKS")) : 64;
-            int sc4 = std::max(1, std::min({max_chunks > 0 ? max_chunks / 2 : target4, total_steps, 256}));
-            const int spc4 = (total_steps + sc4 - 1) / sc4;
-            sc4 = (total_steps + spc4 - 1) / spc4;
+        const Wx4Plan q4 = wgrad4_plan(h, n_evals, M, Nx, Bpad, max_chunks);
+        if (q4.ok) {
+            const int sc4 = q4.sc4, spc4 = q4.spc4, feed = q4.feed;
             if ((size_t)(*chunk_cursor + sc4) * (size_t)len > h->bw.slab_floats) { h->err = "weight-gradient slab overflow"; return RNDE_ERR_BAD_ARG; }
             static constexpr decltype(&rnde_wgrad4x_kernel<true, 0>) kern4[2][2] = {{rnde_wgrad4x_kernel<false, 0>, rnde_wgrad4x_kernel<false, 1>},
                                                                                     {rnde_wgrad4x_kernel<true, 0>, rnde_wgrad4x_kernel<true, 1>}};
@@ -113,13 +132,6 @@
                 attr4.done();
             }
             const dim3 g4(32 * ((sc4 + 7) / 8));
-#if RNDE_WX4_ABL == 7 || RNDE_WX4_ABL == 8
-            const bool q0 = true;
-#else
-            const char* ef = getenv("RNDE_X3_WGRAD_FEED");
-            const bool q0 = getenv("RNDE_X3_WGRAD_Q0") != nullptr || (ef ? ef[0] == '0' : kWx4DefaultFeed == 0);
-#endif
-            const int feed = q0 ? 0 : 1;
             hipLaunchKernelGGL(kern4[tall][feed], g4, dim3(448), lds4[feed], s, ev, n_evals, spc4, sc4, M, Nx, Bpad, dst);
             HIPCHK(h, hipGetLastError());
             *chunk_cursor += sc4;
@@ -158,6 +170,32 @@
     }
     HIPCHK(h, hipGetLastError());
     *chunk_cursor += chunks;
+    return RNDE_OK;
+}
+static rnde_status launch_wgrad_pair(rnde_node* h, const EvalDesc* ev1, const EvalDesc* ev2, int n_evals, int per_chunk, int Bpad, float* slab1, int* cur1,
+                                     float* slab2, int* cur2, hipStream_t s) {
+    const int H = h->H, D = h->D;
+    const Wx4Plan q1 = wgrad4_plan(h, n_evals, H, D, Bpad, 0), q2 = wgrad4_plan(h, n_evals, D, H, Bpad, 0);
+    const long long len1 = (long long)H * (D + 2), len2 = (long long)D * (H + 2);
+    const int most = std::max({q1.sc4, q2.sc4, std::min({128, n_evals * ((Bpad + 31) / 32), 256})});
+    const bool fits = (size_t)(*cur1 + most) * (size_t)len1 <= h->bw.slab_floats && (size_t)(*cur2 + most) * (size_t)len2 <= h->bw.slab_floats;
+    static const bool chunks_env = getenv("RNDE_WGRAD3_CHUNKS") != nullptr;
+    if (!(q1.ok && q2.ok && q1.feed == 1 && q2.feed == 1 && fits && !chunks_env && tail_switch("RNDE_WGRAD_PAIR"))) {
+        rnde_status r = launch_wgrad_part(h, ev1, n_evals, per_chunk, H, D, Bpad, slab1, cur1, s);
+        if (r != RNDE_OK) return r;
+        return launch_wgrad_part(h, ev2, n_evals, per_chunk, D, H, Bpad, slab2, cur2, s);
+    }
+    static DeviceOnce attrp;
+    if (attrp.need()) {
+        HIPCHK(h, hipFuncSetAttribute((const void*)rnde_wgrad4x_pair_kernel, hipFuncAttributeMaxDynamicSharedMemorySize, (int)kWx4fLdsBytes));
+        attrp.done();
+    }
+    const Wx4Job j1{ev1, n_evals, q1.spc4, q1.sc4, H, D, slab1 + (size_t)(*cur1) * len1};
+    const Wx4Job j2{ev2, n_evals, q2.spc4, q2.sc4, D, H, slab2 + (size_t)(*cur2) * len2};
+    const int g1 = 32 * ((q1.sc4 + 7) / 8), g2 = 32 * ((q2.sc4 + 7) / 8);
+    hipLaunchKernelGGL(rnde_wgrad4x_pair_kernel, dim3(g1 + g2), dim3(448), kWx4fLdsBytes, s, j1, j2, g1, Bpad);
+    HIPCHK(h, hipGetLastError());
+    *cur1 += q1.sc4; *cur2 += q2.sc4; ++h->tail_folds[1];
     return RNDE_OK;
 }
 
@@ -235,7 +273,7 @@
             HIPCHK(h, hipEventRecord(ev, s));
             HIPCHK(h, hipStreamWaitEvent(h->wstream, ev, 0));
             ws = h->wstream; used_side = true;
-        }
+        } else return launch_wgrad_pair(h, d_ev1 + lo, d_ev2 + lo, hi - lo, per_chunk, h->B, slab1, &cur1, slab2w, &cur2, s);
         rnde_status r = launch_wgrad_part(h, d_ev1 + lo, hi - lo, per_chunk, h->H, h->D, h->B, slab1, &cur1, ws, on_side ? 16 : 0);
         if (r != RNDE_OK) return r;
         return launch_wgrad_part(h, d_ev2 + lo, hi - lo, per_chunk, h->D, h->H, h->B, slab2w, &cur2, ws, on_side ? 16 : 0);
@@ -319,7 +357,20 @@
         }
         HIPCHK(h, hipGetLastError());
         {
-            for (int step = 0; step < 4; ++step) {
+            const bool pairs = h->persist == 1 && tail_switch("RNDE_BINIT_PAIR");
+            if (pairs) {
+                static constexpr decltype(&rnde_binit_pair_kernel<0, 1>) kPair[2][2] = {{rnde_binit_pair_kernel<0, 1>, rnde_binit_pair_kernel<0, 2>},
+                                                                                      {rnde_binit_pair_kernel<1, 1>, rnde_binit_pair_kernel<1, 2>}};
+                PersistSync Y{h->tslab, h->pabort, h->pxcc, h->persist_spins};
+                HIPCHK(h, slab_prepare(h, Q.F.Bpad, s));
+                const dim3 pgrid(8 * BQ.R * ((BQ.C + 7) / 8));
+                for (int ph = 0; ph < 2; ++ph) {
+                    hipLaunchKernelGGL(kPair[a2][ph], pgrid, blk, h->stage_lds, s, BQ, Y);
+                    ++h->tail_folds[3];
+                    if ((st = couple_sum(h, Q.ipart + ph * 4LL * Q.F.nwg, 4LL * Q.F.nwg, s)) != RNDE_OK) return st;
+                }
+            }
+            for (int step = 0; step < 4 && !pairs; ++step) {
                 hipLaunchKernelGGL(kInit[a2][step], grid, blk, h->stage_lds, s, BQ);
                 if ((step & 1) && (st = couple_sum(h, Q.ipart + (step / 2) * 4LL * Q.F.nwg, 4LL * Q.F.nwg, s)) != RNDE_OK) return st;
             }
@@ -341,10 +392,16 @@
         float* r1 = b.slab_r; float* r2 = b.slab_r + 16 * seg_r;
         const int pg1 = (cur1 + 15) / 16, g1 = (cur1 + pg1 - 1) / pg1, pg2 = (cur2 + 15) / 16, g2 = (cur2 + pg2 - 1) / pg2;
         const int grid = (int)std::min<long long>((std::max(len1, len2) + 255) / 256, 2048);
-        ReducePair A{{{slab1, r1, len1, cur1, pg1}, {slab2w, r2, len2, cur2, pg2}}};
-        hipLaunchKernelGGL(rnde_wgrad_reduce_pair, dim3(grid, std::max(g1, g2), 2), dim3(256), 0, s, A);
-        ReducePair Bp{{{r1, p_bar_dev, len1, g1, g1}, {r2, p_bar_dev + (size_t)h->H * (h->D + 2), len2, g2, g2}}};
-        hipLaunchKernelGGL(rnde_wgrad_reduce_pair, dim3(grid, 1, 2), dim3(256), 0, s, Bp);
+        if (tail_switch("RNDE_REDUCE_FOLD")) {
+            ReducePair F{{{slab1, p_bar_dev, len1, cur1, pg1}, {slab2w, p_bar_dev + (size_t)h->H * (h->D + 2), len2, cur2, pg2}}};
+            hipLaunchKernelGGL(rnde_wgrad_reduce_fold_pair, dim3(grid, 1, 2), dim3(256), 0, s, F);
+            ++h->tail_folds[0];
+        } else {
+            ReducePair A{{{slab1, r1, len1, cur1, pg1}, {slab2w, r2, len2, cur2, pg2}}};
+            hipLaunchKernelGGL(rnde_wgrad_reduce_pair, dim3(grid, std::max(g1, g2), 2), dim3(256), 0, s, A);
+            ReducePair Bp{{{r1, p_bar_dev, len1, g1, g1}, {r2, p_bar_dev + (size_t)h->H * (h->D + 2), len2, g2, g2}}};
+            hipLaunchKernelGGL(rnde_wgrad_reduce_pair, dim3(grid, 1, 2), dim3(256), 0, s, Bp);
+        }
         HIPCHK(h, hipGetLastError());
     } else {
         HIPCHK(h, launch_wgrad_reduce(slab1, cur1, (long long)h->H * (h->D + 2), b.slab_r, p_bar_dev, s));
diff --git a/regneuralde.jl_amd/csrc/rnde_stage.h b/regneuralde.jl_amd/csrc/rnde_stage.h
--- a/regneuralde.jl_amd/csrc/rnde_stage.h
+++ b/regneuralde.jl_amd/csrc/rnde_stage.h
@@ -1,5 +1,6 @@
 #pragma once
 #include "rnde_fwd.h"
+#include "rnde_x3.h"
 
 namespace rnde {
 
@@ -59,11 +60,12 @@
 }
 
 struct PackJob { void* dst; const float* src; long long total; int kind, which, kdim, pad; };
-struct PackJobs { PackJob j[8]; };
+struct PackJobs { PackJob j[8]; X3PackDst x3; int MT, WT, R, HT; };
 static __global__ void rnde_pack_all_kernel(const float* __restrict__ p, const PackJobs J, int D, int H) {
     const PackJob job = J.j[blockIdx.y];
     for (long long i = blockIdx.x * (long long)blockDim.x + threadIdx.x; i < job.total; i += (long long)gridDim.x * blockDim.x) {
         if (job.kind == 0) ((f32x4*)job.dst)[i] = stage_pack_elem(p, job.which, D, H, job.kdim, i);
+        else if (job.kind == 4) x3_pack_elem(p, J.x3, D, H, J.MT, J.WT, J.R, J.HT, i);
         else if (job.kind == 2) ((float*)job.dst)[i] = (job.src ? job.src : p)[i];
         else ((f32x4*)job.dst)[i] = ((const f32x4*)(job.src ? job.src : p))[i];
     }
diff --git a/regneuralde.jl_amd/csrc/rnde_wgradx.h b/regneuralde.jl_amd/csrc/rnde_wgradx.h
--- a/regneuralde.jl_amd/csrc/rnde_wgradx.h
+++ b/regneuralde.jl_amd/csrc/rnde_wgradx.h
@@ -156,13 +156,13 @@
 constexpr int kWx4DefaultFeed = 1;
 
 template <bool TALL_IS_Z, int FEED>
-__global__ __launch_bounds__(448) void rnde_wgrad4x_kernel(const EvalDesc* __restrict__ evals, int n_evals, int per_chunk, int n_chunks, int M, int Nx, int Bpad,
-                                                           float* __restrict__ slab) {
+__device__ __forceinline__ void wgrad4x_body(const int lin, const EvalDesc* __restrict__ evals, int n_evals, int per_chunk, int n_chunks, int M, int Nx, int Bpad,
+                                             float* __restrict__ slab) {
     constexpr int KC = 32;
     extern __shared__ __attribute__((aligned(16))) unsigned short wxs[];
     const int tid = threadIdx.x, lane = tid & 63, w = __builtin_amdgcn_readfirstlane(tid >> 6);
     const int mrow = lane & 15, kk = lane >> 4;
-    const int lin = blockIdx.x, xcd = lin & 7, within = lin >> 3;
+    const int xcd = lin & 7, within = lin >> 3;
     const int chunk = (within >> 2) * 8 + xcd, part = within & 3;
     if (chunk >= n_chunks) return;
     const int TR = TALL_IS_Z ? M : Nx + 2, SR = TALL_IS_Z ? Nx + 2 : M;
@@ -344,5 +344,16 @@
         }
     }
 }
-
-}
+template <bool TALL_IS_Z, int FEED>
+__global__ __launch_bounds__(448) void rnde_wgrad4x_kernel(const EvalDesc* __restrict__ evals, int n_evals, int per_chunk, int n_chunks, int M, int Nx, int Bpad,
+                                                           float* __restrict__ slab) {
+    wgrad4x_body<TALL_IS_Z, FEED>(blockIdx.x, evals, n_evals, per_chunk, n_chunks, M, Nx, Bpad, slab);
+}
+struct Wx4Job { const EvalDesc* evals; int n_evals, per_chunk, n_chunks, M, Nx; float* slab; };
+static __global__ __launch_bounds__(448) void rnde_wgrad4x_pair_kernel(const Wx4Job j1, const Wx4Job j2, const int grid1, const int Bpad) {
+    const int lin = blockIdx.x;
+    if (lin < grid1) wgrad4x_body<false, 1>(lin, j1.evals, j1.n_evals, j1.per_chunk, j1.n_chunks, j1.M, j1.Nx, Bpad, j1.slab);
+    else wgrad4x_body<true, 1>(lin - grid1, j2.evals, j2.n_evals, j2.per_chunk, j2.n_chunks, j2.M, j2.Nx, Bpad, j2.slab);
+}
+
+}
diff --git a/regneuralde.jl_amd/csrc/rnde_x3.h b/regneuralde.jl_amd/csrc/rnde_x3.h
--- a/regneuralde.jl_amd/csrc/rnde_x3.h
+++ b/regneuralde.jl_amd/csrc/rnde_x3.h
@@ -81,14 +81,14 @@
 }
 
 struct X3PackDst { x3u4* d[4]; };
-static __global__ void rnde_x3_pack_kernel(const float* __restrict__ p, const X3PackDst dst, int D, int H, int MT, int WT, int R, int HT) {
+__host__ __device__ __forceinline__ long long x3_pack_count(const X3PackDst& dst, int MT, int R, int HT) { return (dst.d[2] ? 2 : 1) * ((long long)MT * 4 * 64 + (long long)HT * R * 4 * 64); }
+__device__ __forceinline__ void x3_pack_elem(const float* __restrict__ p, const X3PackDst& dst, int D, int H, int MT, int WT, int R, int HT, long long i) {
     const float* W1 = p;
     const float* b1 = W1 + (size_t)H * (D + 1);
     const float* W2 = b1 + H;
     const float* b2 = W2 + (size_t)D * (H + 1);
     const long long nB = (long long)MT * 4 * 64, nD = (long long)HT * R * 4 * 64, per = nB + nD;
-    const int nimg = dst.d[2] ? 2 : 1;
-    for (long long i = blockIdx.x * (long long)blockDim.x + threadIdx.x; i < nimg * per; i += (long long)gridDim.x * blockDim.x) {
+    {
         const int rev = (int)(i / per);
         const long long ii = i - rev * per;
         const bool isD = ii >= nB;
@@ -124,5 +124,9 @@
         o[128] = (x3u4){lo[0], lo[1], lo[2], lo[3]};
     }
 }
+static __global__ void rnde_x3_pack_kernel(const float* __restrict__ p, const X3PackDst dst, int D, int H, int MT, int WT, int R, int HT) {
+    const long long total = x3_pack_count(dst, MT, R, HT);
+    for (long long i = blockIdx.x * (long long)blockDim.x + threadIdx.x; i < total; i += (long long)gridDim.x * blockDim.x) x3_pack_elem(p, dst, D, H, MT, WT, R, HT, i);
+}
 
 }
```

Result: faster. 318,100 samples/s (median of 6 runs) (+1.0%).
